# michiyasunaga/qagnn

Hardware: AMD Instinct MI355X
Metric: QA-subgraphs/sec (batch x num_choice) fwd+bwd (higher is better)
Workload: dtype f32; 1 GPU; configs[1]: CSQA-shaped batch 64 questions x 5 choices = 320 subgraphs per GPU, n=200 node slots, 400..2000 edges/subgraph, 38 relations (run_qagnn__csqa.sh), 5-layer GAT d=200 H=4, QAGNN decoder fwd+bwd (LM encoder excluded: random sent_vecs), dropout 0.2, train-mode BN; subgraphs_per_gpu=320, nodes=64000, edges=396800, edges_with_self_loops=460800, graph_input=load-time int32 blobs (qagnn_graph_from_blobs), 13.3 B/edge on the wire, parallelism=single

## Files before the change

__graft_entry__.py:

```python
import os
import sys

ROOT = os.path.dirname(os.path.abspath(__file__))
if ROOT not in sys.path:
    sys.path.insert(0, ROOT)


def build():
    from qagnn_amd.build import build as build_lib
    path = build_lib(force=False)
    from qagnn_amd import _lib
    lib = _lib.load_library(path)
    assert lib.qagnn_abi_version() == _lib.ABI_VERSION
    for name in _lib.EXPORTS + _lib.EXPORTS_TN + _lib.EXPORTS_INFER + _lib.EXPORTS_LOSS + _lib.EXPORTS_EXPLAIN:
        assert hasattr(lib, name), name
    import qagnn_amd.modeling_qagnn
    import oracle.qagnn_oracle
    print(f'[build] {path} ok ({os.path.getsize(path)} bytes), {len(_lib.EXPORTS)} C-ABI symbols')


def smoke():
    import torch
    sys.path.insert(0, os.path.join(ROOT, 'tests'))
    import helpers
    from qagnn_amd import modeling_qagnn as MQ
    from qagnn_amd import ops
    assert torch.cuda.is_available(), 'smoke() needs an MI355X'
    torch.set_num_threads(min(os.cpu_count() or 1, 32))
    case = dict(shape='config1', nq=1, nc=5, n=100, n_rel=17, std=0.6, train=True, seed=3,
                cfg=helpers.model_cfg(d=200, k=5, sent_dim=64, n_concept=1000, concept_in_dim=32))
    cfg = case['cfg']
    inp = helpers.make_case_inputs(case)
    B, n = 5, 100
    args = [inp['sent_vecs'], inp['concept_ids'].view(B, n), inp['node_type_ids'].view(B, n), inp['node_scores'].view(B, n, 1),
            inp['adj_lengths'].view(B), inp['edge_index'], inp['edge_type']]
    torch.manual_seed(0)
    model = MQ.QAGNN(None, cfg['k'], 4, 38, cfg['sent_dim'], cfg['n_concept'], 200, cfg['concept_in_dim'], 2, 200, 0, 0.0, 0.0, 0.0)
    helpers.det_fill_(model, 3, 0.6)
    model.pooler.dropout.p = model.pooler.attention.dropout.p = 0.0
    model = model.train().to('cuda:0')
    dargs = [a.to('cuda:0') for a in args]
    with helpers.recorded_forward(cfg['concept_dim']) as relu_in:
        logits, attn = model(*dargs[:5], (dargs[5], dargs[6]))
    (logits * torch.linspace(0.5, 1.5, B, device='cuda:0').view(B, 1)).sum().backward()
    assert ops.kernels().name == 'hip'
    ref = helpers.F64Ref(case, 'grad', inputs=tuple(args))
    ref.compute_yard()
    dl = helpers._close(logits.detach().cpu(), ref.forward32['::logits'], rtol=1e-4, atol=1e-5, what='logits')
    da = helpers._close(attn.detach().cpu(), ref.forward32['::pool_attn'], rtol=1e-4, atol=1e-5, what='pool_attn')
    report = ref.check_all({k: p.grad for k, p in model.named_parameters() if p.grad is not None}, what='smoke grad::', min_checked=60,
                           **helpers.kink_args(relu_in, cfg, args[5], args[6], args[2]))
    worst = max(report, key=report.get)
    print(f'[smoke] logits max|d| = {dl:.3e}, pool_attn max|d| = {da:.3e}; {len(report)} gradient tensors on the float64 yardstick, '
          f'worst {report[worst]:.2e} of scale ({worst})')


if __name__ == '__main__':
    build()
    if len(sys.argv) > 1 and sys.argv[1] == 'smoke':
        smoke()
```

qagnn_amd/_lib.py:

```python
import ctypes as C
import functools
import os

import torch

_HERE = os.path.dirname(os.path.abspath(__file__))
LIB_PATH = os.environ.get('QAGNN_LIB') or os.path.join(_HERE, 'libqagnn_hip.so')

EXPORTS = ['qagnn_last_error', 'qagnn_abi_version', 'qagnn_graph_storage_elems', 'qagnn_graph_prep', 'qagnn_graph_prep_blocked',
           'qagnn_graph_from_blobs', 'qagnn_radam_step_f32', 'qagnn_node_prep_f32', 'qagnn_seed_epoch_advance', 'qagnn_seed_epoch_set',
           'qagnn_gemm_nn_f32', 'qagnn_gemm_nn_split_f32', 'qagnn_gemm_nn_pack_bytes', 'qagnn_gemm_nn_ws_bytes', 'qagnn_gemm_nn_split_ws_f32', 'qagnn_gemm_nn_prepack_bytes', 'qagnn_gemm_nn_prepack_f32',
           'qagnn_gemm_nn_prepack_clear', 'qagnn_gemm_tn_workspace_elems', 'qagnn_gemm_tn_f32', 'qagnn_gemm_tn2_f32', 'qagnn_gemm_tn_colsum_f32',
           'qagnn_colreduce_workspace_elems', 'qagnn_colreduce_f32', 'qagnn_bn_finalize_f32', 'qagnn_bn_stats_finalize_f32', 'qagnn_bn_relu_bwd_f32',
           'qagnn_gelu_dropout_fwd_f32', 'qagnn_gelu_dropout_bwd_f32', 'qagnn_sin_basis_f32',
           'qagnn_bn_relu_bwd_colsum_f32',
           'qagnn_pool_attn_fwd_f32', 'qagnn_pool_attn_bwd_f32', 'qagnn_head_post_fwd_f32', 'qagnn_head_post_bwd_f32', 'qagnn_add_row0_f32', 'qagnn_gather_multi_f32', 'qagnn_gather_multi_sum_f32',
           'qagnn_edge_attn_fwd_f32', 'qagnn_edge_attn_bwd_f32',
           'qagnn_hop_fwd_workspace_elems', 'qagnn_hop_bwd_workspace_elems', 'qagnn_hop_fwd_f32', 'qagnn_hop_bwd_f32',
           'qagnn_stack_fwd_f32', 'qagnn_stack_bwd_f32', 'qagnn_absmax_f32', 'qagnn_zero_words', 'qagnn_gemm_tn_h2_f32', 'qagnn_gelu_dropout_fwd_amax_f32', 'qagnn_gelu_dropout_amax_scratch_elems',
           'qagnn_timing_enable', 'qagnn_timing_read', 'qagnn_gemm_tn_h1_f32', 'qagnn_gelu_dropout_bwd_amax_f32', 'qagnn_packed_min_rows',
           'qagnn_radam_step_scaled_f32', 'qagnn_grad_norm_workspace_elems', 'qagnn_grad_norm_f32', 'qagnn_scale_multi_f32', 'qagnn_graph_prep_cap',
           'qagnn_store_gather', 'qagnn_graph_from_store']
EXPORTS_TN = ['qagnn_gemm_tn_graph_f32', 'qagnn_gemm_tn_route_query', 'qagnn_tn_work_table', 'qagnn_tn_live_tiles']
EXPORTS_INFER = ['qagnn_infer_version', 'qagnn_bn_relu_absmax_scratch_elems', 'qagnn_bn_relu_absmax_f32', 'qagnn_stack_infer_f32',
                 'qagnn_choice_eval_f32']
EXPORTS_LOSS = ['qagnn_loss_version', 'qagnn_choice_loss_f32', 'qagnn_choice_loss_bwd_f32']
EXPORTS_EXPLAIN = ['qagnn_explain_version', 'qagnn_attn_export_f32', 'qagnn_attn_trace_f32']
TRACE_MAX_N = 1024
LOSS_KINDS = {'cross_entropy': 0, 'margin_rank': 1}
LOSS_THREADS = 256

CLS_SLICES = 4
ABI_VERSION = 25

_i32, _i64, _f32, _u64, _vp = C.c_int32, C.c_int64, C.c_float, C.c_uint64, C.c_void_p


class qagnn_graph(C.Structure):
    _fields_ = ([(n, _i32) for n in ('N', 'E', 'Ep', 'R', 'T', 'C')] +
                [(n, _vp) for n in ('rowptr_s', 'tgt_s', 'src_s', 'cls_s', 'eid_s', 'rowptr_t', 'src_t', 'tgt_t', 'cls_t', 'pos_t',
                                    'cls_count', 'src_c', 'tgt_c', 'pos_c', 'chunk_cls', 'chunk_beg',
                                    'chunk_len', 'n_chunks', 'chunkptr')] +
                [('max_chunks', _i32), ('err', _vp), ('block_n', _i32), ('n_groups', _i32)])


class qagnn_store(C.Structure):
    _fields_ = ([(n, _vp) for n in ('blobs', 'blob_off', 'concept_ids', 'node_type', 'node_scores', 'adj_len')] +
                [('S', _i32), ('n', _i32), ('W', _i64)])


GATHER_MAX = 160


class qagnn_gather_tabs(C.Structure):
    _fields_ = [('p', _vp * GATHER_MAX), ('n', _i32)]


class qagnn_pack_desc(C.Structure):
    _fields_ = [('B1n', _vp), ('ldn1', _i32), ('K1', _i32), ('B2n', _vp), ('ldn2', _i32), ('K2', _i32), ('No', _i32), ('pieces', _i32)]


class qagnn_gemm_nn_args(C.Structure):
    _fields_ = [('A1', _vp), ('lda1', _i32), ('K1', _i32), ('B1', _vp), ('ldb1', _i32),
                ('A2', _vp), ('lda2', _i32), ('K2', _i32), ('B2', _vp), ('ldb2', _i32),
                ('C', _vp), ('ldc', _i32), ('M', _i32), ('No', _i32),
                ('bias', _vp), ('rowtab', _vp), ('ldt', _i32), ('rowidx', _vp),
                ('a_scale', _vp), ('a_shift', _vp), ('accumulate', _i32), ('a_rowidx', _vp), ('xcd_remap', _i32), ('colstat_part', _vp),
                ('a_amax1', _vp), ('a_amax2', _vp), ('a_rows', _i64), ('pieces', _i32)]


class qagnn_hop_args(C.Structure):
    _fields_ = ([('g', C.POINTER(qagnn_graph))] + [(n, _i32) for n in ('N', 'DP', 'SP', 'HP', 'T')] + [('qscale', _f32)] +
                [(n, _vp) for n in ('X', 'S', 'ntype', 'Wx_t', 'Wx', 'Ws_t', 'Ws', 'TT', 'EkEm', 'W1t', 'W1', 'b1', 'gamma', 'beta',
                                    'W2t', 'W2', 'b2')] +
                [('batch_stats', _i32), ('eps', _f32), ('run_mean_p', _vp), ('run_var_p', _vp), ('run_mean', _vp), ('run_var', _vp),
                 ('num_batches_tracked', _vp), ('dense_pos', _vp), ('d', _i32), ('momentum', _f32),
                 ('apply_act', _i32), ('p_drop', _f32), ('seed', _u64)] +
                [(n, _vp) for n in ('KMQ', 'a', 'alpha', 'aggr', 'h1', 'out', 'y', 'stats', 'dy', 'dX', 'dS')] +
                [('accumulate_dS', _i32), ('accumulate_dX', _i32)] +
                [(n, _vp) for n in ('dWx_t', 'dWs_t', 'dTT', 'dEkEm', 'dW1t', 'db1', 'dbn', 'dW2t', 'db2', 'ws')] +
                [('ws_elems', _i64), ('gemm_split', _i32), ('ones_col', _i32), ('tab_col', _i32), ('side_stream', _vp), ('amax', _vp), ('x_amax', _vp), ('s_amax', _vp)])


HOP_AMAX_WORDS = 16
HOP_AM_X, HOP_AM_S, HOP_AM_AGGR, HOP_AM_H1, HOP_AM_Y, HOP_AM_DOUT, HOP_AM_DH1, HOP_AM_DKMQ = range(8)


def load_library(path=LIB_PATH):
    if not os.path.exists(path):
        raise OSError(f'{path} not found: build it with `python -m qagnn_amd.build` (hipcc, gfx950)')
    lib = C.CDLL(path)
    lib.qagnn_last_error.restype = C.c_char_p
    lib.qagnn_abi_version.restype = _i32
    lib.qagnn_graph_storage_elems.restype = _i64
    lib.qagnn_graph_storage_elems.argtypes = [_i32, _i32, _i32, _i32]
    lib.qagnn_graph_prep.argtypes = [C.POINTER(qagnn_graph), _vp, _vp, _vp, _vp, _i32, _i32, _i32, _i32, _vp]
    lib.qagnn_graph_prep_blocked.argtypes = [C.POINTER(qagnn_graph), _vp, _vp, _vp, _vp, _i32, _i32, _i32, _i32, _i32, _vp]
    lib.qagnn_graph_prep_cap.argtypes = [C.POINTER(qagnn_graph), _vp, _vp, _i64, _vp, _vp, _i32, _i32, _vp, _i32, _i32, _i32, _vp]
    lib.qagnn_graph_from_blobs.argtypes = [C.POINTER(qagnn_graph), _vp, _vp, _vp, _vp, _vp, _i32, _i32, _i32, _i32, _i32, _vp]
    lib.qagnn_store_gather.argtypes = [C.POINTER(qagnn_store), _vp, _i32, _vp, _vp, _vp, _vp, _vp, _vp, _vp]
    lib.qagnn_graph_from_store.argtypes = [C.POINTER(qagnn_graph), _vp, C.POINTER(qagnn_store), _vp, _vp, _vp, _i32, _i32, _i32, _i32, _vp]
    lib.qagnn_node_prep_f32.argtypes = [_vp, _vp, _vp, _vp, _i32, _i32, _vp, _vp, _vp, _i64, _vp, _vp]
    lib.qagnn_seed_epoch_advance.argtypes = [_u64, _vp]
    lib.qagnn_seed_epoch_set.argtypes = [_u64, _vp]
    lib.qagnn_radam_step_f32.argtypes = [_i32, _vp, _vp, _vp, _vp, _vp] + [C.c_double] * 6 + [_i32, _vp]
    lib.qagnn_radam_step_scaled_f32.argtypes = [_i32, _vp, _vp, _vp, _vp, _vp] + [C.c_double] * 6 + [_i32, _vp, _vp]
    lib.qagnn_grad_norm_workspace_elems.restype = _i64
    lib.qagnn_grad_norm_workspace_elems.argtypes = [_i32, _vp]
    lib.qagnn_grad_norm_f32.argtypes = [_i32, _vp, _vp, C.c_double, _vp, _vp, _vp]
    lib.qagnn_scale_multi_f32.argtypes = [_i32, _vp, _vp, _vp, _vp]
    lib.qagnn_gemm_nn_f32.argtypes = [C.POINTER(qagnn_gemm_nn_args), _vp]
    lib.qagnn_gemm_nn_split_f32.argtypes = [C.POINTER(qagnn_gemm_nn_args), _vp, _i32, _vp, _i32, _vp]
    lib.qagnn_gemm_nn_pack_bytes.restype = _i64
    lib.qagnn_gemm_nn_pack_bytes.argtypes = [_i32, _i32, _i32]
    lib.qagnn_gemm_nn_split_ws_f32.argtypes = [C.POINTER(qagnn_gemm_nn_args), _vp, _i32, _vp, _i32, _vp, _i64, _vp]
    lib.qagnn_gemm_nn_ws_bytes.restype = _i64
    lib.qagnn_gemm_nn_ws_bytes.argtypes = [C.POINTER(qagnn_gemm_nn_args), _vp, _i32, _vp, _i32]
    lib.qagnn_gemm_nn_prepack_bytes.restype = _i64
    lib.qagnn_gemm_nn_prepack_bytes.argtypes = [C.POINTER(qagnn_pack_desc), _i32]
    lib.qagnn_gemm_nn_prepack_f32.argtypes = [C.POINTER(qagnn_pack_desc), _i32, _vp, _i64, _i64, _vp]
    lib.qagnn_gemm_nn_prepack_clear.argtypes = [_i64]
    lib.qagnn_gemm_tn_workspace_elems.restype = _i64
    lib.qagnn_gemm_tn_workspace_elems.argtypes = [_i32, _i32, _i32]
    lib.qagnn_gemm_tn_f32.argtypes = [_vp, _i32, _vp, _i32, _vp, _i32, _i32, _i32, _i32, _vp, _vp, _vp, _i32, _vp, _vp]
    lib.qagnn_gemm_tn2_f32.argtypes = [_vp, _i32, _i32, _vp, _i32, _i32, _vp, _i32, _vp, _i32, _i32, _i32, _vp, _vp]
    lib.qagnn_gemm_tn_h2_f32.argtypes = [_vp, _i32, _i32, _vp, _i32, _i32, _vp, _i32, _vp, _i32, _i32, _i32, _vp, _vp, _vp, _vp, _vp, _vp, _vp]
    lib.qagnn_gemm_tn_h1_f32.argtypes = lib.qagnn_gemm_tn_h2_f32.argtypes
    lib.qagnn_gemm_tn_graph_f32.argtypes = [_vp, _i32, _i32, _vp, _i32, _i32, _vp, _i32, _vp, _i32, _i32, _i32, _vp, _vp, _vp, _i32,
                                            C.POINTER(qagnn_graph), _vp, _vp]
    lib.qagnn_gemm_tn_route_query.argtypes = [_i32, _i32, _i32, _i32, _vp]
    lib.qagnn_tn_work_table.argtypes = [C.POINTER(qagnn_graph), _i32, _i32, _vp, _vp]
    lib.qagnn_tn_live_tiles.argtypes = [_i32]
    lib.qagnn_absmax_f32.argtypes = [_vp, _i64, _vp, _vp]
    lib.qagnn_zero_words.argtypes = [_vp, _i64, _vp]
    lib.qagnn_timing_enable.argtypes = [_i32]
    lib.qagnn_timing_read.argtypes = [_vp, _vp]
    lib.qagnn_packed_min_rows.restype = _i64
    lib.qagnn_packed_min_rows.argtypes = [_i64]
    lib.qagnn_gemm_tn_colsum_f32.argtypes = [_vp, _i32, _vp, _i32, _vp, _i32, _i32, _i32, _i32, _vp, _vp, _vp, _i32, _vp, _vp, _i32,
                                             _vp, _vp]
    lib.qagnn_colreduce_workspace_elems.restype = _i64
    lib.qagnn_colreduce_workspace_elems.argtypes = [_i32, _i32, _i32]
    lib.qagnn_colreduce_f32.argtypes = [_i32, _vp, _i32, _vp, _i32, _i32, _i32, _vp, _i32, _vp, _vp, _vp, _vp, _vp, _f32, _vp, _vp, _vp]
    lib.qagnn_bn_finalize_f32.argtypes = [_vp, _vp, _vp, _vp, _f32, _vp, _vp, _vp, _i32, _vp, _vp, _vp, _vp, _i32, _f32, _f32, _i32, _vp]
    lib.qagnn_bn_stats_finalize_f32.argtypes = [_vp, _i32, _i32, _i32, _vp, _vp, _f32, _vp, _vp, _vp, _vp, _vp, _i32, _f32, _f32, _i32, _vp]
    lib.qagnn_bn_relu_bwd_f32.argtypes = [_vp, _vp, _vp, _i32, _i32, _i32, _vp, _vp, _vp, _vp, _vp, _vp, _vp, _f32, _vp, _vp]
    lib.qagnn_gelu_dropout_fwd_f32.argtypes = [_vp, _vp, _i64, _f32, _u64, _vp]
    lib.qagnn_gelu_dropout_bwd_f32.argtypes = [_vp, _vp, _vp, _i64, _f32, _u64, _vp]
    lib.qagnn_gelu_dropout_fwd_amax_f32.argtypes = [_vp, _vp, _i64, _f32, _u64, _vp, _vp, _vp]
    lib.qagnn_gelu_dropout_bwd_amax_f32.argtypes = [_vp, _vp, _vp, _i64, _f32, _u64, _vp, _vp, _vp]
    lib.qagnn_gelu_dropout_amax_scratch_elems.restype = _i64
    lib.qagnn_gelu_dropout_amax_scratch_elems.argtypes = [_i64]
    lib.qagnn_sin_basis_f32.argtypes = [_vp, _vp, _vp, _i32, _i32, _i32, _vp]
    lib.qagnn_bn_relu_bwd_colsum_f32.argtypes = [_vp, _vp, _vp, _i32, _i32, _i32, _vp, _vp, _vp, _vp, _vp, _vp, _vp, _f32, _vp, _vp, _vp, _vp]
    lib.qagnn_pool_attn_fwd_f32.argtypes = [_vp, _vp, _vp, _i32, _vp, _i32, _i32, _i32, _i32, _f32, _f32, _u64, _vp, _vp, _vp, _vp]
    lib.qagnn_pool_attn_bwd_f32.argtypes = [_vp, _vp, _i32, _i32, _i32, _i32, _i32, _f32, _f32, _u64, _vp, _vp, _vp, _vp, _vp, _i32, _vp, _vp, _vp]
    lib.qagnn_head_post_fwd_f32.argtypes = [_vp, _vp, _vp, _vp, _vp, _vp, _i64, _vp, _vp, _i32, _i32, _i32, _i32, _i32, _i32, _i32, _f32, _f32, _u64, _u64,
                                            _vp, _vp, _vp, _vp]
    lib.qagnn_head_post_bwd_f32.argtypes = [_vp, _vp, _vp, _vp, _vp, _vp, _vp, _i64, _vp, _i32, _i32, _i32, _i32, _i32, _i32, _i32, _f32, _f32, _u64, _u64,
                                            _vp, _vp, _vp, _vp, _vp, _vp, _i32, _vp]
    lib.qagnn_add_row0_f32.argtypes = [_vp, _i64, _vp, _i32, _i32, _vp]
    lib.qagnn_gather_multi_f32.argtypes = [C.POINTER(qagnn_gather_tabs), _vp, _vp, _vp, _i32, _vp]
    lib.qagnn_gather_multi_sum_f32.argtypes = [C.POINTER(qagnn_gather_tabs), _vp, _vp, _i32, _i32, _vp, _vp]
    lib.qagnn_edge_attn_fwd_f32.argtypes = [C.POINTER(qagnn_graph), _vp, _i32, _vp, _i32, _i32, _f32, _vp, _vp, _vp, _vp, _i32, _vp]
    lib.qagnn_edge_attn_bwd_f32.argtypes = [C.POINTER(qagnn_graph), _vp, _i32, _vp, _i32, _i32, _f32, _vp, _vp, _vp, _i32,
                                            _vp, _vp, _vp, _vp, _vp, _vp]
    lib.qagnn_hop_fwd_workspace_elems.restype = _i64
    lib.qagnn_hop_fwd_workspace_elems.argtypes = [_i32, _i32, _i32]
    lib.qagnn_hop_bwd_workspace_elems.restype = _i64
    lib.qagnn_hop_bwd_workspace_elems.argtypes = [_i32, _i32, _i32, _i32, _i32]
    lib.qagnn_hop_fwd_f32.argtypes = [C.POINTER(qagnn_hop_args), _vp]
    lib.qagnn_hop_bwd_f32.argtypes = [C.POINTER(qagnn_hop_args), _vp]
    lib.qagnn_stack_fwd_f32.argtypes = [C.POINTER(qagnn_hop_args), _i32, _vp]
    lib.qagnn_stack_bwd_f32.argtypes = [C.POINTER(qagnn_hop_args), _i32, _vp]
    lib.qagnn_infer_version.argtypes = []
    lib.qagnn_bn_relu_absmax_scratch_elems.restype = _i64
    lib.qagnn_bn_relu_absmax_scratch_elems.argtypes = [_i32, _i32]
    lib.qagnn_bn_relu_absmax_f32.argtypes = [_vp, _i32, _i32, _i32, _vp, _vp, _vp, _vp, _vp]
    lib.qagnn_stack_infer_f32.argtypes = [C.POINTER(qagnn_hop_args), _i32, _vp]
    lib.qagnn_choice_eval_f32.argtypes = [_vp, _i64, _vp, _i32, _i32, _vp, _vp, _vp]
    lib.qagnn_loss_version.argtypes = []
    lib.qagnn_choice_loss_f32.argtypes = [_vp, _i64, _vp, _i32, _i32, _i32, _f32, _vp, _vp, _vp, _i64, _vp, _vp, _vp]
    lib.qagnn_choice_loss_bwd_f32.argtypes = [_vp, _i64, _vp, _vp, _i64, _i32, _i32, _vp]
    lib.qagnn_explain_version.argtypes = []
    lib.qagnn_attn_export_f32.argtypes = [C.POINTER(qagnn_graph), _vp, _i64, _i32, _vp, _i64, _vp]
    lib.qagnn_attn_trace_f32.argtypes = [C.POINTER(qagnn_graph), _vp, _i64, _i32, _i32, _i32, _i32, _i32, _vp, _vp, _vp, _vp]
    for name in EXPORTS + EXPORTS_TN + EXPORTS_INFER + EXPORTS_LOSS + EXPORTS_EXPLAIN:
        fn = getattr(lib, name)
        if fn.restype is C.c_int and name not in ('qagnn_abi_version',):
            fn.restype = _i32
    return lib


def _ptr(t):
    return None if t is None else t.data_ptr()


def choice_loss_bound(kind, nc, Q, max_abs=1.0, margin=0.0, weight=1.0, threads=LOSS_THREADS):
    import math
    u, v = 2.0 ** -24, 2.0 ** -53
    M, L, w = max(1.0, float(max_abs)), math.log(nc), abs(float(weight))
    S = -(-Q // threads) + math.log2(threads) + nc
    if LOSS_KINDS[kind] == 0:
        return w * M * (u * (nc + 8 + 5 * L) + v * S * (2 + L)), w / Q * u * (nc + 8 + L)
    return w * M * (3 * u + v * S) * (2 + abs(float(margin)) / M), w / Q * 2 * u


def _running_fields(running):
    if running is None:
        return None, None, None, None, 0, 0.0, 1.0
    rm, rv, nbt, pos, mom, unb = running
    assert rm.is_contiguous() and rv.is_contiguous() and pos.dtype == torch.long and (nbt is None or nbt.dtype == torch.long)
    return rm.data_ptr(), rv.data_ptr(), _ptr(nbt), pos.data_ptr(), rm.numel(), float(mom), float(unb)


def _chk2d(t, name, dtype=torch.float32):
    assert t.is_cuda and t.dtype == dtype and t.dim() == 2 and t.is_contiguous(), \
        f'{name}: need a contiguous 2-D {dtype} device tensor, got {tuple(t.shape)} {t.dtype} {t.device}'
    return t


def _chkp(t, name):
    assert t.is_cuda and t.dtype == torch.float32 and t.dim() == 2, f'{name}: need a 2-D float32 device tensor, got {tuple(t.shape)} {t.dtype} {t.device}'
    assert t.is_contiguous() or (t.stride(1) == 1 and (t.size(0) == 1 or (t.stride(0) >= t.size(1) and t.stride(0) % 4 == 0)) and t.data_ptr() % 16 == 0), \
        f'{name}: rows must be contiguous, a multiple of 4 floats (and at least their width) apart and 16-byte aligned; got strides {t.stride()} for {tuple(t.shape)}'
    return t


def _ld(t):
    return t.size(1) if t.size(0) == 1 else t.stride(0)


def _chkp3(t, name):
    assert t.is_cuda and t.dtype == torch.float32 and t.dim() == 3, f'{name}: need a 3-D float32 device tensor'
    B, n, Cc = t.shape
    ld = _ld3(t)
    assert t.is_contiguous() or (t.stride(2) == 1 and ld >= Cc and ld % 4 == 0 and (B == 1 or t.stride(0) == n * ld) and t.data_ptr() % 16 == 0), \
        f'{name}: need [B, n, Cc] rows with one pitch (a multiple of 4 floats, >= Cc), 16-byte aligned; got strides {t.stride()} for {tuple(t.shape)}'
    return t


def _ld3(t):
    B, n, Cc = t.shape
    return t.stride(1) if n > 1 else (t.stride(0) if B > 1 else Cc)


VALIDATE = os.environ.get('QAGNN_VALIDATE', '0') == '1'


class _ErrWatch:

    def __init__(self):
        self.pending = []
        self.sink = None

    def watch(self, flags, what, reset=None):
        if torch.cuda.is_current_stream_capturing():
            if self.sink is not None:
                self.sink.append((flags, what, reset))
            return
        self.after_replay([(flags, what, reset)])

    def after_replay(self, watched):
        for flags, what, reset in watched:
            host = torch.empty(4, dtype=torch.int32, pin_memory=True)
            host.copy_(flags, non_blocking=True)
            ev = torch.cuda.Event()
            ev.record()
            self.pending.append((ev, host, what, reset))
        if VALIDATE:
            self.poll(block=True)

    def poll(self, block=False):
        if torch.cuda.is_available() and torch.cuda.is_current_stream_capturing():
            return
        keep, bad = [], None
        for ev, host, what, reset in self.pending:
            if block:
                ev.synchronize()
            if not ev.query():
                keep.append((ev, host, what, reset))
            elif int(host[0]) != 0:
                if reset is not None:
                    reset.zero_()
                if bad is None:
                    bad = what
        self.pending = keep
        if bad is not None:
            raise RuntimeError(f'out-of-range input in {bad}: the device replaced it by a safe value; the results of that batch '
                               'are not the reference\'s (which raises in its one-hot / index ops)')


ERR_WATCH = _ErrWatch()


class HipGraph:

    def __init__(self, storage, cstruct, N, E, R, T, block_n=0):
        self.storage, self.c = storage, cstruct
        self.N, self.E, self.Ep, self.R, self.T = N, E, E + N, R, T
        self.block_n = block_n
        self.dynamic = False
        self.C = R * T * T + T
        self.max_chunks = cstruct.max_chunks

    def array(self, name, length):
        off = (getattr(self.c, name) - self.storage.data_ptr()) // 4
        return self.storage[off:off + length]

    def live_tiles(self):
        T = (self.N + 31) // 32
        T4 = (T + 3) // 4 * 4
        w = self.array('err', 16 + 4 + 2 * T4)[16:]
        return w[4:4 + T], w[4 + T4:4 + T4 + T], w[:1]

    @property
    def cls_part_rows(self):
        return self.max_chunks + CLS_SLICES * self.C

    @property
    def cls_count(self):
        return self.array('cls_count', self.C)

    @property
    def eid_s(self):
        return self.array('eid_s', self.Ep)


def _device_of(args, kwargs):
    for a in list(args) + list(kwargs.values()):
        if isinstance(a, torch.Tensor):
            if a.is_cuda:
                return a.device
        elif isinstance(a, HipGraph):
            return a.storage.device
        elif isinstance(a, (tuple, list)):
            for t in a:
                if isinstance(t, torch.Tensor) and t.is_cuda:
                    return t.device
    return None


def _on_operand_device(fn):
    @functools.wraps(fn)
    def wrapped(self, *args, **kwargs):
        dev = _device_of(args, kwargs)
        if dev is None or dev.index == torch.cuda.current_device():
            return fn(self, *args, **kwargs)
        with torch.cuda.device(dev):
            return fn(self, *args, **kwargs)
    return wrapped


class _GuardedMeta(type):
    def __new__(mcls, name, bases, ns):
        for k, v in list(ns.items()):
            if callable(v) and not k.startswith('_'):
                ns[k] = _on_operand_device(v)
        return super().__new__(mcls, name, bases, ns)


class HipKernels(metaclass=_GuardedMeta):
    name = 'hip'
    infer_attn = True
    tn_live = True

    def __init__(self):
        if not torch.cuda.is_available():
            raise RuntimeError('qagnn_amd needs an MI355X: torch.cuda.is_available() is False and there is no CPU fallback')
        self.lib = load_library()
        if self.lib.qagnn_abi_version() != ABI_VERSION:
            raise RuntimeError('libqagnn_hip.so ABI version mismatch')
        self.gemm_split = {'0': 0, '1': 1, '3': 3}.get(os.environ.get('QAGNN_GEMM_SPLIT', '2'), 2)
        self.PACK_MIN_M = int(self.lib.qagnn_packed_min_rows(-1))
        self._side_streams = {}
        self._loss_flags = {}

    def _stream(self):
        return torch._C._cuda_getCurrentRawStream(torch.cuda.current_device())

    def _side_stream(self):
        dev = torch.cuda.current_device()
        st = self._side_streams.get(dev)
        if st is None:
            st = self._side_streams[dev] = torch.cuda.Stream(device=dev)
        return st.cuda_stream

    def _check(self, rc, what):
        if rc != 0:
            raise RuntimeError(f'{what} failed (code {rc}): {self.lib.qagnn_last_error().decode()}')

    def _graph_alloc(self, N, E, R, T, device, storage=None):
        elems = self.lib.qagnn_graph_storage_elems(N, E, R, T)
        if storage is None:
            storage = torch.empty(elems, dtype=torch.int32, device=device)
        assert storage.is_cuda and storage.dtype == torch.int32 and storage.is_contiguous() and storage.numel() >= elems
        return storage, qagnn_graph()
# ... 804 lines not shown
        self._check_scale_word(grad_out, g.device)
        Q, nc = g.shape
        if out is None:
            out = torch.empty((Q, nc), dtype=torch.float32, device=g.device)
        assert out.dtype == torch.float32 and out.shape == (Q, nc) and out.device == g.device and (out.stride(1) == 1 or nc == 1)
        self._check(self.lib.qagnn_choice_loss_bwd_f32(g.data_ptr(), _ld(g), grad_out.data_ptr(), out.data_ptr(), _ld(out), Q, nc, self._stream()),
                    'qagnn_choice_loss_bwd_f32')
        return out

    def stack_infer(self, graph, HP, qscale, X, S, ntype, prms, eps, cols=-1, x_amax=None, s_amax=None, keep=False, attn=False):
        assert not (keep and attn)
        k = len(prms)
        N, DP, Ep, dev = graph.N, 4 * HP, graph.Ep, X.device
        kk = k if keep else 1
        KMQ = torch.empty((kk, N, 3 * DP), dtype=torch.float32, device=dev)
        aa = torch.empty((kk, 2, Ep, 4), dtype=torch.float32, device=dev)
        rows = torch.empty((kk, 4, N, DP), dtype=torch.float32, device=dev) if keep else torch.empty((5, N, DP), dtype=torch.float32, device=dev)
        stats = torch.empty((kk, 5, DP), dtype=torch.float32, device=dev)
        amax = torch.empty((k, HOP_AMAX_WORDS), dtype=torch.int32, device=dev)
        ws = self._fwd_ws(graph, DP, dev)
        ys = [rows[l, 3] if keep else rows[3 + (l & 1)] for l in range(k)]
        hops = self._hop_chain(graph, HP, qscale, X, S, ntype, prms, ys, (KMQ, aa, rows, stats), amax.data_ptr(), x_amax, s_amax, ws, False, eps, 0.0,
                               None, cols, shared=not keep)
        if attn:
            a_all = torch.empty((k, Ep, 4), dtype=torch.float32, device=dev)
            for l in range(k):
                hops[l].a = a_all.data_ptr() + l * Ep * 16
        self._check(self.lib.qagnn_stack_infer_f32(hops, k, self._stream()), 'qagnn_stack_infer_f32')
        if attn:
            return ys[-1], amax, a_all
        return (ys[-1], amax, (KMQ, aa, rows, stats)) if keep else (ys[-1], amax)

    @staticmethod
    def _chk_attn(graph, a):
        assert a.is_cuda and a.dtype == torch.float32 and a.dim() == 3 and a.shape[1:] == (graph.Ep, 4), \
            f'a: need a [k, Ep = {graph.Ep}, 4] float32 device tensor, got {tuple(a.shape)} {a.dtype} {a.device}'
        k = a.size(0)
        ls = a.stride(0) if k > 1 else 4 * graph.Ep
        assert k == 0 or ((graph.Ep == 1 or a.stride(1) == 4) and a.stride(2) == 1 and ls >= 4 * graph.Ep and ls % 4 == 0 and a.data_ptr() % 16 == 0), \
            f'a: rows of 4 contiguous floats, layers a multiple of 4 floats apart, 16-byte aligned; got strides {a.stride()}'
        return k, ls

    def attn_export(self, graph, a, out=None):
        k, ls = self._chk_attn(graph, a)
        if out is None:
            out = torch.empty((k, graph.Ep, 4), dtype=torch.float32, device=a.device)
        ko, ols = self._chk_attn(graph, out)
        assert ko == k and out.device == a.device
        self._check(self.lib.qagnn_attn_export_f32(C.byref(graph.c), a.data_ptr() if k else None, ls, k, out.data_ptr() if k else None, ols,
                                                   self._stream()), 'qagnn_attn_export_f32')
        return out

    def attn_trace(self, graph, a, B, n, root=0, head=-1, out=None):
        k, ls = self._chk_attn(graph, a)
        N, dev = graph.N, a.device
        if out is None:
            out = (torch.empty((k + 1, N), dtype=torch.float32, device=dev), torch.empty((k + 1, N), dtype=torch.float32, device=dev),
                   torch.empty((k, N), dtype=torch.int32, device=dev))
        flow, best, pred = out
        for t, rows, dt in ((flow, k + 1, torch.float32), (best, k + 1, torch.float32), (pred, k, torch.int32)):
            assert t.is_cuda and t.dtype == dt and t.shape == (rows, N) and t.is_contiguous() and t.device == dev
        self._check(self.lib.qagnn_attn_trace_f32(C.byref(graph.c), a.data_ptr() if k else None, ls, k, int(B), int(n), int(root), int(head),
                                                  flow.data_ptr(), best.data_ptr(), pred.data_ptr() if k else None, self._stream()),
                    'qagnn_attn_trace_f32')
        return flow, best, pred

    def stack_fwd(self, graph, HP, qscale, X, S, ntype, prms, batch_stats, eps, p, seeds, runnings, cols=-1, x_amax=None, s_amax=None):
        k = len(prms)
        N, DP, Ep, dev = graph.N, 4 * HP, graph.Ep, X.device
        KMQ = torch.empty((k, N, 3 * DP), dtype=torch.float32, device=dev)
        aa = torch.empty((k, 2, Ep, 4), dtype=torch.float32, device=dev)
        rows = torch.empty((k, 4, N, DP), dtype=torch.float32, device=dev)
        stats = torch.empty((k, 5, DP), dtype=torch.float32, device=dev)
        amax = torch.empty((k, HOP_AMAX_WORDS), dtype=torch.int32, device=dev)
        ws = self._fwd_ws(graph, DP, dev)
        ys = rows[:, 3].unbind(0)
        hops = self._hop_chain(graph, HP, qscale, X, S, ntype, prms, ys, (KMQ, aa, rows, stats), amax.data_ptr(), x_amax, s_amax, ws, batch_stats, eps, p,
                               seeds, cols, runnings=runnings)
        self._check(self.lib.qagnn_stack_fwd_f32(hops, k, self._stream()), 'qagnn_stack_fwd_f32')
        ext = torch.empty(0, dtype=torch.int32, device=dev)
        return ys[k - 1], (KMQ, aa, rows, stats, amax, x_amax if x_amax is not None else ext, s_amax if s_amax is not None else ext)

    def stack_bwd(self, graph, HP, qscale, X, S, ntype, prms, batch_stats, eps, p, seeds, saved, dy, need_dX, need_dS, dX_acc=None, tab_col=-1,
                  overlap=True):
        k = len(prms)
        KMQ, aa, rows, stats = saved[:4]
        p_amax = saved[4].data_ptr() if len(saved) > 4 else None
        x_amax, s_amax = (saved[5], saved[6]) if len(saved) > 6 else (None, None)
        N, DP, Ep, dev = graph.N, 4 * HP, graph.Ep, X.device
        SP = S.size(1) if S is not None else 0
        _chk2d(dy, 'dy')
        sizes, offs = self._grad_sizes(DP, SP, prms[0][4].size(0), graph.C)
        per = offs[-1]
        flat = torch.empty(k * per, dtype=torch.float32, device=dev)
        dxs = torch.empty((max(k - 1, 1), N, DP), dtype=torch.float32, device=dev)
        dS = torch.empty((N, SP), dtype=torch.float32, device=dev) if (SP and need_dS) else None
        dX = None
        if need_dX:
            dX = dX_acc if dX_acc is not None else torch.empty((N, DP), dtype=torch.float32, device=dev)
            assert dX.shape == (N, DP) and dX.is_contiguous()
        ws = self._bwd_ws(graph, DP, SP, dev)
        hops = self._hop_chain(graph, HP, qscale, X, S, ntype, prms, rows[:, 3].unbind(0), (KMQ, aa, rows, stats), p_amax, x_amax, s_amax, ws,
                               batch_stats, eps, p, seeds, tab_col, side=overlap)
        grads, p_dxs, row_b = [], dxs.data_ptr(), N * DP * 4
        for l, h in enumerate(hops):
            h.dy = dy.data_ptr() if l == k - 1 else p_dxs + l * row_b
            grads.append(self._carve_grads(h, flat[l * per:(l + 1) * per], sizes, offs, graph.C))
            if l > 0:
                h.dX, h.accumulate_dX = p_dxs + (l - 1) * row_b, 0
            elif dX is not None:
                h.dX, h.accumulate_dX = dX.data_ptr(), (1 if dX_acc is not None else 0)
            if dS is not None:
                h.dS, h.accumulate_dS = dS.data_ptr(), (0 if l == k - 1 else 1)
        self._check(self.lib.qagnn_stack_bwd_f32(hops, k, self._stream()), 'qagnn_stack_bwd_f32')
        return dX, dS, grads
```

qagnn_amd/build.py:

```python
import hashlib
import os
import subprocess
import sys

HERE = os.path.dirname(os.path.abspath(__file__))
CSRC = os.path.join(HERE, 'csrc')
LIB = os.path.join(HERE, 'libqagnn_hip.so')
STAMP = LIB + '.srchash'
SOURCES = ['graph_prep.hip', 'gemm.hip', 'elementwise.hip', 'edge_attn.hip', 'pool.hip', 'hop.hip', 'optim.hip', 'gemm_split.hip', 'gemm_nn2.hip', 'gemm_dispatch.hip', 'timing.hip', 'infer.hip', 'loss.hip', 'explain.hip']
FLAGS = ['--offload-arch=gfx950', '-O3', '-std=c++17', '-fPIC', '-shared']


def hashed_files():
    headers = sorted(f for f in os.listdir(CSRC) if f.endswith('.h'))
    return [os.path.join(CSRC, s) for s in SOURCES + headers] + [os.path.join(HERE, '..', 'include', 'qagnn_hip.h'),
                                                                 os.path.join(HERE, '..', 'include', 'qagnn_hip_tn.h'),
                                                                 os.path.join(HERE, '..', 'include', 'qagnn_hip_infer.h'),
                                                                 os.path.join(HERE, '..', 'include', 'qagnn_hip_loss.h'),
                                                                 os.path.join(HERE, '..', 'include', 'qagnn_hip_explain.h')]


def source_hash():
    h = hashlib.sha256(' '.join(FLAGS).encode())
    for p in hashed_files():
        with open(p, 'rb') as f:
            h.update(os.path.basename(p).encode() + b'\0' + f.read() + b'\0')
    return h.hexdigest()


def up_to_date():
    if not (os.path.exists(LIB) and os.path.exists(STAMP)):
        return False
    with open(STAMP) as f:
        return f.read().strip() == source_hash()


def build(force=False, verbose=True):
    if not force and up_to_date():
        return LIB
    hipcc = os.environ.get('HIPCC', '/opt/rocm/bin/hipcc')
    cmd = [hipcc] + FLAGS + ['-o', LIB] + [os.path.join(CSRC, s) for s in SOURCES]
    if verbose:
        print(' '.join(cmd), flush=True)
    if os.path.exists(STAMP):
        os.remove(STAMP)
    subprocess.check_call(cmd)
    with open(STAMP, 'w') as f:
        f.write(source_hash() + '\n')
    return LIB


if __name__ == '__main__':
    print(build(force='--force' in sys.argv))
```

qagnn_amd/csrc/common.h:

```cpp
#pragma once
#include <hip/hip_runtime.h>
#include <stdint.h>
#include <stdio.h>

#include <type_traits>

#include "../../include/qagnn_hip.h"
#include "../../include/qagnn_hip_tn.h"
#include "../../include/qagnn_hip_infer.h"

namespace qagnn {

void set_error(const char* fmt, ...);

struct NnProduct {
  const qagnn_gemm_nn_args* a;
  bool split;
  const float* B1n; int ldn1; const float* B2n; int ldn2;
  void* ws; int64_t ws_bytes;
};
enum class NnFamily { FP32, SPLIT, NN2 };
enum class NnB { IN_KERNEL, PACK, IMAGE };
struct NnRoute {
  NnFamily family;
// ... 36 lines not shown
  const float* a_scale; const float* a_shift; const int64_t* a_rowidx; int accumulate;
  float* bsum; const int64_t* b_rowidx; int groups;
  const uint32_t* amax[3]; int np;
  float* ws;
  const qagnn_graph* g;
};
inline TnProduct tn_product(const float* A1, int lda1, int Ka1, const float* A2, int lda2, int Ka2, const float* B, int ldb, float* C, int ldc, int R,
                            int No, const float* a_scale, const float* a_shift, float* ws, const uint32_t* amax_a1 = nullptr,
                            const uint32_t* amax_a2 = nullptr, const uint32_t* amax_b = nullptr, int np = 3) {
  TnProduct p = {};
  p.A1 = A1; p.lda1 = lda1; p.Ka1 = Ka1;
  if (A2 && Ka2 > 0) { p.A2 = A2; p.lda2 = lda2; p.Ka2 = Ka2; p.two = true; }
  p.B = B; p.ldb = ldb; p.C = C; p.ldc = ldc; p.R = R; p.No = No; p.a_scale = a_scale; p.a_shift = a_shift; p.ws = ws;
  p.amax[0] = amax_a1; p.amax[1] = amax_a2; p.amax[2] = amax_b; p.np = np;
  return p;
}
enum class TnFamily { RUNTIME, STRIP, SPLIT, WS, PAIR };
struct TnRoute {
  TnFamily family;
  int kt, nt, waves, np;
  bool affine, gather, colsum;
  int chunk_rows, nchunks;
  bool sum_by4;
  bool live;
  dim3 grid;
  int64_t ws_elems;
};
TnRoute tn_route(const TnProduct& p);
int gemm_tn(const TnProduct& p, hipStream_t stream);
int launch_tn(const TnRoute& r, const TnProduct& p, float* Pcs, hipStream_t stream);
int launch_tn_strip(const TnRoute& r, const TnProduct& p, float* Pcs, hipStream_t stream);
int launch_tn_split(const TnRoute& r, const TnProduct& p, hipStream_t stream);
int launch_tn_ws(const TnRoute& r, const TnProduct& p, hipStream_t stream);
int launch_sum_chunks(const float* P, float* C, int ldc, int rows, int No, int nchunks, int accumulate, bool by4, hipStream_t stream);

constexpr int TN_LIST_CAP = 1024;
constexpr int TN_LIVE_BC = 208;
struct TnLive { const int* list; const int* n_live; int T, S, chunk_tiles; };
struct TnWork { int cK, cM, lenM, qK, rK; };
struct TnSlot { int cb, list, beg, cnt, pslot; };
__host__ __device__ inline TnWork tn_work(int S, int T, int L, int chunk_tiles) {
  TnWork w;
  L = L < 0 ? 0 : (L > T ? T : L);
  if (L >= T) {
    w.cK = S / 3; w.cM = S - 2 * w.cK; w.lenM = chunk_tiles; w.qK = -1; w.rK = 0;
    return w;
  }
  const long long den = (long long)T + 2ll * L;
  int c = (int)((2ll * S * L + den) / (2 * den));
  const int hi = (S - 1) / 2;
  c = c < 1 ? 1 : (c > hi ? hi : c);
  w.cK = c; w.cM = S - 2 * c; w.lenM = (T + w.cM - 1) / w.cM; w.qK = L / c; w.rK = L % c;
  return w;
}
__host__ __device__ inline TnSlot tn_slot(const TnWork& w, int S, int T, int u) {
  auto start = [&](int j) { return 2 * j + (int)((long long)j * w.cM / w.cK); };
  int j = (int)((long long)u * w.cK / S);
  while (j > 0 && start(j) > u) --j;
  while (j + 1 < w.cK && start(j + 1) <= u) ++j;
  const int off = u - start(j);
  TnSlot s;
  auto range = [&](int i) { s.list = 0; s.beg = i * w.lenM < T ? i * w.lenM : T; s.cnt = T - s.beg < w.lenM ? T - s.beg : w.lenM; };
  if (off < 2) {
    s.cb = off == 0 ? 0 : 2;
    s.pslot = off == 0 ? j : w.cK + j;
    if (w.qK < 0) range(j);
    else { s.list = 1; s.beg = j * w.qK + (j < w.rK ? j : w.rK); s.cnt = w.qK + (j < w.rK ? 1 : 0); }
  } else {
    const int m = (int)((long long)j * w.cM / w.cK) + off - 2;
    s.cb = 1;
    s.pslot = 2 * w.cK + m;
    range(m);
  }
  return s;
}
int launch_sum_chunks_live(const float* P, float* C, int ldc, int rows, const TnLive& lv, int accumulate, hipStream_t stream);
bool tn_live_enabled();
struct LiveTiles { int n_tiles; int32_t *n_live, *live, *list; };
inline LiveTiles live_tiles_of(const qagnn_graph* g) {
  const int T = (int)(((int64_t)g->N + 31) / 32), T4 = (T + 3) & ~3;
  int32_t* const p = g->err + 16;
  return LiveTiles{T, p, p + 4, p + 4 + T4};
}

int launch_gelu_dropout(const float* X, const float* dY, float* out, int64_t n, float p, uint64_t seed, uint32_t* amax, float* amax_part,
                        hipStream_t stream);
int64_t gelu_amax_scratch_elems(int64_t n);
int launch_bn_relu_bwd_colsum(const float* dR, const float* Hh, float* dH, int ld, int R, int Cc, const float* mean, const float* invstd,
                              const float* scale, const float* shift, const float* gamma, const float* sum_dy, const float* sum_dy_hhat,
                              float inv_rows, const float* roww, float* colsum, float* workspace, uint32_t* amax, hipStream_t stream);
int launch_bn_stats_finalize(const float* part, int n_tiles, int R, int Cc, const float* gamma, const float* beta, float eps, float* stats,
                             float* run_mean, float* run_var, int64_t* nbt, int d, float momentum, float unbias, int ones_col, uint32_t* amax_bound,
                             hipStream_t stream);

int launch_edge_attn_fwd(const qagnn_graph* g, const float* KMQ, int32_t ldk, const float* EkEm, int32_t lde, int32_t HP, float qscale,
                         float* score, float* a, float* alpha, float* aggr, int32_t lda, float* amax_part , hipStream_t stream);
int launch_edge_attn_bwd(const qagnn_graph* g, const float* KMQ, int32_t ldk, const float* EkEm, int32_t lde, int32_t HP, float qscale,
                         const float* a, const float* alpha, const float* G, int32_t ldg, float* dKMQ, float* dEkEm, float* ga, float* rs,
                         float* cls_part, float* amax_part , uint32_t* amax_slot, hipStream_t stream);
int launch_amax_reduce(const float* part, int64_t n, uint32_t* slot, hipStream_t stream);
int launch_bn_relu_absmax(const float* H, int ldh, int R, int Cc, const float* scale, const float* shift, uint32_t* slot, float* part, hipStream_t stream);

struct TimedScope {
  int kind;
  hipStream_t s;
  hipEvent_t e0, e1;
  bool counted;
  TimedScope(int kind, hipStream_t s);
  ~TimedScope();
  TimedScope(const TimedScope&) = delete;
  TimedScope& operator=(const TimedScope&) = delete;
};

#define QAGNN_REQUIRE(cond, code, ...) \
  do {                                 \
    if (!(cond)) {                     \
      qagnn::set_error(__VA_ARGS__);   \
      return (code);                   \
    }                                  \
  } while (0)

#define QAGNN_LAUNCH_CHECK(name)                                               \
  do {                                                                         \
    hipError_t e__ = hipGetLastError();                                        \
    if (e__ != hipSuccess) {                                                   \
      qagnn::set_error("%s launch failed: %s", name, hipGetErrorString(e__));  \
      return QAGNN_EHIP;                                                       \
    }                                                                          \
  } while (0)

#ifndef QAGNN_NN_OCC
#define QAGNN_NN_OCC 2
#endif

template <int V0, int... Vs, class F>
inline int dispatch_int(int v, F&& f) {
  if constexpr (sizeof...(Vs) == 0) return f(std::integral_constant<int, V0>{});
  else return v == V0 ? f(std::integral_constant<int, V0>{}) : dispatch_int<Vs...>(v, f);
}
template <class F>
inline int dispatch_bool(bool v, F&& f) { return v ? f(std::true_type{}) : f(std::false_type{}); }

template <auto KERNEL>
inline int raise_lds_limit(int bytes, const char* name) {
  static bool raised[64] = {};
  int dev = 0;
  if (hipGetDevice(&dev) != hipSuccess) dev = 0;
  if (bytes <= 64 * 1024 || raised[dev & 63]) return QAGNN_OK;
  hipError_t e = hipFuncSetAttribute((const void*)KERNEL, hipFuncAttributeMaxDynamicSharedMemorySize, bytes);
  if (e != hipSuccess) { set_error("%s: cannot raise the dynamic LDS limit: %s", name, hipGetErrorString(e)); return QAGNN_EHIP; }
  raised[dev & 63] = true;
  return QAGNN_OK;
}

static inline bool aligned16(const void* p) { return (reinterpret_cast<uintptr_t>(p) & 15u) == 0; }

__device__ __forceinline__ int xcd_remap(int b, int nblocks) {
  const int q = nblocks >> 3, r = nblocks & 7;
  const int xcd = b & 7, slot = b >> 3;
  const int base = xcd < r ? xcd * (q + 1) : r * (q + 1) + (xcd - r) * q;
  return base + slot;
}

__host__ __device__ __forceinline__ int edge_xcd_cap(int N) {
  const int per = (((N + 3) >> 2) + 7) >> 3;
  return (per * 5 + 3) >> 2;
}
__device__ __forceinline__ int xcd_remap_balanced(int b, const int* __restrict__ base) {
  const int xcd = b & 7, lb = base[xcd] + (b >> 3);
  return lb < base[xcd + 1] ? lb : -1;
}

const unsigned long long* seed_epoch_ptr();
__device__ __forceinline__ uint64_t epoch_seed(uint64_t seed, const unsigned long long* __restrict__ epoch) {
  return epoch ? seed + (uint64_t)epoch[0] * 0xD1B54A32D192ED03ull : seed;
}

__device__ __forceinline__ float uniform01(uint64_t seed, uint64_t idx) {
  uint64_t z = seed + (idx + 1) * 0x9E3779B97F4A7C15ull;
  z = (z ^ (z >> 30)) * 0xBF58476D1CE4E5B9ull;
  z = (z ^ (z >> 27)) * 0x94D049BB133111EBull;
  z = z ^ (z >> 31);
// ... 121 lines not shown
```

qagnn_amd/csrc/edge_attn.hip:

```cpp
#include "common.h"

namespace qagnn {

#ifndef EDGE_UNROLL
#define EDGE_UNROLL 4
#endif
#define TGT_UNROLL 4

typedef __amdgpu_buffer_rsrc_t rsrc_t;
constexpr uint32_t OOB_OFF = 0x7FFFFFF0u;
__device__ __forceinline__ rsrc_t make_rsrc(const void* base, uint32_t bytes) {
  return __builtin_amdgcn_make_buffer_rsrc(const_cast<void*>(base), 0, (int)bytes, 0x00020000);
}
__device__ __forceinline__ float4 buf_ld4(rsrc_t r, uint32_t voff, uint32_t soff) {
  return __builtin_bit_cast(float4, __builtin_amdgcn_raw_buffer_load_b128(r, (int)voff, (int)soff, 0));
}

constexpr int SLAB_ROWS = 72;

struct Lane {
  int lane, w, g, j;
  bool act;
  uint32_t voff;
  int off;
// ... 270 lines not shown
  const int s = wave_node(xcd_base);
  if (s >= N) return;
  const Lane L = lane_info(HP);
  const int DP = 4 * HP;
  const uint32_t pk = (uint32_t)ldk * 4u, pe = (uint32_t)lde * 4u;
  const rsrc_t rK = make_rsrc(KMQ, (uint32_t)N * pk), rE = make_rsrc(EkEm, (uint32_t)C * pe);
  const int beg = __builtin_amdgcn_readfirstlane(rowptr_s[s]), end = __builtin_amdgcn_readfirstlane(rowptr_s[s + 1]);
  if (end - beg == 1) {
    if (L.act) st4(dKMQ + (int64_t)s * ldk + 2 * DP + L.off, zero4());
    if (amax_part && L.lane == 63) amax_part[s] = 0.f;
    return;
  }
  const float4 r4 = ld4(rs + (int64_t)s * 4);
  slab_init(slab[L.w], L.lane);
  const float* const sl = reinterpret_cast<const float*>(slab[L.w]) + L.g;
  float4 dQ = zero4();
  for (int e0 = beg; e0 < end; e0 += 64) {
    const int cnt = min(64, end - e0), lc = e0 + min(L.lane, cnt - 1);
    const uint32_t tv = (uint32_t)tgt_s[lc] * pk, cv = (uint32_t)cls_s[lc] * pe;
    float4 gs4 = zero4();
    if (L.lane < cnt) {
      const float4 a4 = ld4(a + (int64_t)lc * 4), g4 = ld4(ga + (int64_t)lc * 4);
      gs4 = make_float4(qscale * a4.x * (g4.x - r4.x), qscale * a4.y * (g4.y - r4.y), qscale * a4.z * (g4.z - r4.z),
                        qscale * a4.w * (g4.w - r4.w));
      st4(ga + (int64_t)lc * 4, gs4);
    }
    slab[L.w][L.lane] = gs4;
    for (int i = 0; i < cnt; i += EDGE_UNROLL) {
      float4 k[EDGE_UNROLL], ek[EDGE_UNROLL];
#pragma unroll
      for (int u = 0; u < EDGE_UNROLL; ++u) {
        const int idx = min(i + u, cnt - 1);
        k[u] = buf_ld4(rK, L.voff, rl(tv, idx));
        ek[u] = buf_ld4(rE, L.voff, rl(cv, idx));
      }
#pragma unroll
      for (int u = 0; u < EDGE_UNROLL; ++u) dQ = fma4(sl[(i + u) * 4], add4(k[u], ek[u]), dQ);
    }
  }
  if (L.act) st4(dKMQ + (int64_t)s * ldk + 2 * DP + L.off, dQ);
  if (amax_part) node_amax(L.act ? absmax4(dQ) : 0.f, amax_part, s);
}

__global__ __launch_bounds__(256) void k_edge_bwd_tgt(const int* __restrict__ rowptr_t, const int* __restrict__ src_t,
                                                      const int* __restrict__ pos_t, const float* __restrict__ KMQ, int ldk,
                                                      int HP, const float* __restrict__ gsb, float* __restrict__ dKMQ, int N,
                                                      const int* __restrict__ xcd_base, float* __restrict__ amax_part) {
  __shared__ float4 slab[4][SLAB_ROWS];
  const int t = wave_node(xcd_base);
  if (t >= N) return;
  const Lane L = lane_info(HP);
  const int DP = 4 * HP;
  const uint32_t pk = (uint32_t)ldk * 4u, vq = L.voff + 2u * DP * 4u;
  const rsrc_t rK = make_rsrc(KMQ, (uint32_t)N * pk);
  const int beg = __builtin_amdgcn_readfirstlane(rowptr_t[t]), end = __builtin_amdgcn_readfirstlane(rowptr_t[t + 1]);
  if (end - beg == 1) {
    const int sv = __builtin_amdgcn_readfirstlane(src_t[beg]), pv = __builtin_amdgcn_readfirstlane(pos_t[beg]);
    const float4 q1 = buf_ld4(rK, vq, (uint32_t)sv * pk);
    const float gs1 = gsb[(int64_t)pv * 4 + L.g];
    const float4 k1 = fma4(gs1, q1, zero4());
    if (L.act) st4(dKMQ + (int64_t)t * ldk + L.off, k1);
    if (amax_part) node_amax(L.act ? absmax4(k1) : 0.f, amax_part, t);
    return;
  }
  slab_init(slab[L.w], L.lane);
  const float* const sl = reinterpret_cast<const float*>(slab[L.w]) + L.g;
  float4 dK = zero4();
  for (int e0 = beg; e0 < end; e0 += 64) {
    const int cnt = min(64, end - e0), lc = e0 + min(L.lane, cnt - 1);
    const uint32_t sv = (uint32_t)src_t[lc] * pk;
    slab[L.w][L.lane] = L.lane < cnt ? ld4(gsb + (int64_t)pos_t[lc] * 4) : zero4();
    for (int i = 0; i < cnt; i += TGT_UNROLL) {
      float4 qv[TGT_UNROLL];
#pragma unroll
      for (int u = 0; u < TGT_UNROLL; ++u) qv[u] = buf_ld4(rK, vq, rl(sv, min(i + u, cnt - 1)));
#pragma unroll
      for (int u = 0; u < TGT_UNROLL; ++u) dK = fma4(sl[(i + u) * 4], qv[u], dK);
    }
  }
  if (L.act) st4(dKMQ + (int64_t)t * ldk + L.off, dK);
  if (amax_part) node_amax(L.act ? absmax4(dK) : 0.f, amax_part, t);
}

__global__ __launch_bounds__(256) void k_edge_bwd_cls(const int* __restrict__ n_chunks, const int* __restrict__ chunk_beg,
                                                      const int* __restrict__ chunk_len, const int* __restrict__ src_c,
                                                      const int* __restrict__ tgt_c, const int* __restrict__ pos_c,
                                                      const float* __restrict__ KMQ, int ldk, int HP,
                                                      const float* __restrict__ alpha, const float* __restrict__ gsb,
                                                      const float* __restrict__ G, int ldg, float* __restrict__ cls_part, int N) {
  __shared__ float4 slab[2][4][SLAB_ROWS];
  const int nch = *n_chunks, nb_real = (nch + 3) >> 2;
  if ((int)blockIdx.x >= nb_real) return;
  const int k = __builtin_amdgcn_readfirstlane(xcd_remap(blockIdx.x, nb_real) * 4 + (threadIdx.x >> 6));
  if (k >= nch) return;
  const Lane L = lane_info(HP);
  const int DP = 4 * HP;
  const uint32_t pk = (uint32_t)ldk * 4u, pg = (uint32_t)ldg * 4u, vq = L.voff + 2u * DP * 4u;
  const rsrc_t rK = make_rsrc(KMQ, (uint32_t)N * pk), rG = make_rsrc(G, (uint32_t)N * pg);
  const int beg = __builtin_amdgcn_readfirstlane(chunk_beg[k]), len = __builtin_amdgcn_readfirstlane(chunk_len[k]);
  slab_init(slab[0][L.w], L.lane);
  slab_init(slab[1][L.w], L.lane);
  const float* const sl_gs = reinterpret_cast<const float*>(slab[0][L.w]) + L.g;
  const float* const sl_al = reinterpret_cast<const float*>(slab[1][L.w]) + L.g;
  float4 dEk = zero4(), dEm = zero4();
  for (int b0 = 0; b0 < len; b0 += 64) {
    const int cnt = min(64, len - b0), lc = beg + b0 + min(L.lane, cnt - 1);
    const uint32_t sv = (uint32_t)src_c[lc] * pk, tv = (uint32_t)tgt_c[lc] * pg;
    const int pv = pos_c[lc];
    slab[0][L.w][L.lane] = L.lane < cnt ? ld4(gsb + (int64_t)pv * 4) : zero4();
    slab[1][L.w][L.lane] = L.lane < cnt ? ld4(alpha + (int64_t)pv * 4) : zero4();
    for (int i = 0; i < cnt; i += EDGE_UNROLL) {
      float4 qv[EDGE_UNROLL], g4[EDGE_UNROLL];
#pragma unroll
      for (int u = 0; u < EDGE_UNROLL; ++u) {
        const int idx = min(i + u, cnt - 1);
        qv[u] = buf_ld4(rK, vq, rl(sv, idx));
        g4[u] = buf_ld4(rG, L.voff, rl(tv, idx));
      }
#pragma unroll
      for (int u = 0; u < EDGE_UNROLL; ++u) {
        dEk = fma4(sl_gs[(i + u) * 4], qv[u], dEk);
        dEm = fma4(sl_al[(i + u) * 4], g4[u], dEm);
      }
    }
  }
  if (L.act) {
    st4(cls_part + (int64_t)k * 2 * DP + L.off, dEk);
    st4(cls_part + (int64_t)k * 2 * DP + DP + L.off, dEm);
  }
}

__global__ __launch_bounds__(1024) void k_cls_reduce(const int* __restrict__ chunkptr, const float* __restrict__ cls_part,
                                                     float* __restrict__ slices, int DP2, int C, int NG) {
  extern __shared__ float4 sm4[];
  __shared__ int cp_lo[QAGNN_CLS_GROUPS], cp_hi[QAGNN_CLS_GROUPS];
  const int c = blockIdx.x, sl = blockIdx.y;
  if (threadIdx.x < NG) {
    cp_lo[threadIdx.x] = chunkptr[threadIdx.x * C + c];
    cp_hi[threadIdx.x] = chunkptr[threadIdx.x * C + c + 1];
  }
  __syncthreads();
  const int ncol4 = DP2 >> 2;
  const int P = (int)blockDim.x / ncol4;
  const int col4 = threadIdx.x % ncol4, part = threadIdx.x / ncol4;
  float4 acc = zero4();
  if (part < P) {
    int seen = 0;
    for (int g = sl; g < NG; g += QAGNN_CLS_SLICES) {
      const int kb = cp_lo[g], ke = cp_hi[g];
      const int first = (part - seen % P + P) % P;
      for (int k = kb + first; k < ke; k += P) acc = add4(acc, ld4(cls_part + (int64_t)k * DP2 + col4 * 4));
      seen += ke - kb;
    }
    sm4[part * ncol4 + col4] = acc;
  }
  __syncthreads();
  if (threadIdx.x < ncol4) {
    float4 s = sm4[threadIdx.x];
    for (int q = 1; q < P; ++q) s = add4(s, sm4[q * ncol4 + threadIdx.x]);
    st4(slices + ((int64_t)c * QAGNN_CLS_SLICES + sl) * DP2 + threadIdx.x * 4, s);
  }
}
__global__ __launch_bounds__(256) void k_cls_reduce2(const float* __restrict__ slices, float* __restrict__ dEkEm, int lde, int DP2, int C,
                                                     const float* __restrict__ amax_part, int npart, uint32_t* __restrict__ amax_slot) {
  const int ncol4 = DP2 >> 2;
  const int i = blockIdx.x * blockDim.x + threadIdx.x;
  if (i < C * ncol4) {
    const int c = i / ncol4, col4 = i - c * ncol4;
    const float* p = slices + (int64_t)c * QAGNN_CLS_SLICES * DP2 + col4 * 4;
    float4 s = ld4(p);
#pragma unroll
    for (int q = 1; q < QAGNN_CLS_SLICES; ++q) s = add4(s, ld4(p + (int64_t)q * DP2));
    st4(dEkEm + (int64_t)c * lde + col4 * 4, s);
  }
  if (amax_part) {
    __shared__ float red[16];
    float m = 0.f;
    for (int k = i; k < npart; k += (int)(gridDim.x * blockDim.x)) m = fmaxf(m, amax_part[k]);
    block_amax_merge(m, amax_slot, red);
  }
}

static int check_common(const qagnn_graph* g, const float* KMQ, int ldk, const float* EkEm, int lde, int HP, const char* who) {
  QAGNN_REQUIRE(g && KMQ && EkEm, QAGNN_EINVAL, "%s: null pointer", who);
  QAGNN_REQUIRE(HP > 0 && HP % 4 == 0 && HP <= 64, QAGNN_EUNSUPPORTED, "%s: head pitch HP=%d must be a multiple of 4, <= 64", who, HP);
  QAGNN_REQUIRE(ldk >= 12 * HP && ldk % 4 == 0 && lde >= 8 * HP && lde % 4 == 0, QAGNN_EINVAL, "%s: ldk=%d lde=%d too small for HP=%d",
                who, ldk, lde, HP);
  QAGNN_REQUIRE(aligned16(KMQ) && aligned16(EkEm), QAGNN_EINVAL, "%s: operands must be 16-byte aligned", who);
  QAGNN_REQUIRE((int64_t)g->N * ldk * 4 < (int64_t)OOB_OFF && (int64_t)g->C * lde * 4 < (int64_t)OOB_OFF, QAGNN_EUNSUPPORTED,
                "%s: N=%d x ldk=%d floats exceed the 2 GiB a buffer descriptor of these kernels addresses", who, g->N, ldk);
  return QAGNN_OK;
}

}

using namespace qagnn;

namespace qagnn {
int launch_edge_attn_fwd(const qagnn_graph* g, const float* KMQ, int32_t ldk, const float* EkEm, int32_t lde, int32_t HP, float qscale,
                         float* score, float* a, float* alpha, float* aggr, int32_t lda, float* amax_part, hipStream_t stream) {
  TimedScope timed(2, stream);
  int rc = check_common(g, KMQ, ldk, EkEm, lde, HP, "edge_attn_fwd");
  if (rc != QAGNN_OK) return rc;
  QAGNN_REQUIRE(score && a && alpha && aggr && lda >= 4 * HP && lda % 4 == 0 && aligned16(aggr), QAGNN_EINVAL,
                "edge_attn_fwd: bad output arguments");
  const int nb = 8 * edge_xcd_cap(g->N);
  k_edge_scores<<<nb, 256, 0, stream>>>(g->rowptr_s, g->tgt_s, g->cls_s, KMQ, ldk, EkEm, lde, HP, qscale, score, a, alpha, g->N, g->C, g->err + 4);
  QAGNN_LAUNCH_CHECK("k_edge_scores");
  k_edge_aggregate<<<nb, 256, 0, stream>>>(g->rowptr_t, g->src_t, g->cls_t, g->pos_t, KMQ, ldk, EkEm, lde, HP, alpha, aggr, lda, g->N, g->C, g->err + 4, amax_part);
  QAGNN_LAUNCH_CHECK("k_edge_aggregate");
  return QAGNN_OK;
}
}

extern "C" int qagnn_edge_attn_fwd_f32(const qagnn_graph* g, const float* KMQ, int32_t ldk, const float* EkEm, int32_t lde,
                                       int32_t HP, float qscale, float* score, float* a, float* alpha, float* aggr, int32_t lda,
                                       qagnn_stream_t stream_) {
  return launch_edge_attn_fwd(g, KMQ, ldk, EkEm, lde, HP, qscale, score, a, alpha, aggr, lda, nullptr, (hipStream_t)stream_);
}

extern "C" int qagnn_edge_attn_bwd_f32(const qagnn_graph* g, const float* KMQ, int32_t ldk, const float* EkEm, int32_t lde,
                                       int32_t HP, float qscale, const float* a, const float* alpha, const float* G, int32_t ldg,
                                       float* dKMQ, float* dEkEm, float* ga, float* rs, float* cls_part, qagnn_stream_t stream_) {
  return launch_edge_attn_bwd(g, KMQ, ldk, EkEm, lde, HP, qscale, a, alpha, G, ldg, dKMQ, dEkEm, ga, rs, cls_part, nullptr, nullptr, (hipStream_t)stream_);
}

int qagnn::launch_edge_attn_bwd(const qagnn_graph* g, const float* KMQ, int32_t ldk, const float* EkEm, int32_t lde, int32_t HP, float qscale,
                                const float* a, const float* alpha, const float* G, int32_t ldg, float* dKMQ, float* dEkEm, float* ga, float* rs,
                                float* cls_part, float* amax_part, uint32_t* amax_slot, hipStream_t stream) {
  TimedScope timed(3, stream);
  int rc = check_common(g, KMQ, ldk, EkEm, lde, HP, "edge_attn_bwd");
  if (rc != QAGNN_OK) return rc;
  QAGNN_REQUIRE(a && alpha && G && dKMQ && dEkEm && ga && rs && cls_part, QAGNN_EINVAL, "edge_attn_bwd: null pointer");
  QAGNN_REQUIRE(ldg >= 4 * HP && ldg % 4 == 0 && aligned16(G) && aligned16(dKMQ) && aligned16(dEkEm) && aligned16(cls_part),
                QAGNN_EINVAL, "edge_attn_bwd: bad pitch / alignment");
  QAGNN_REQUIRE((int64_t)g->N * ldg * 4 < (int64_t)OOB_OFF, QAGNN_EUNSUPPORTED, "edge_attn_bwd: G exceeds 2 GiB");
  const int DP2 = 8 * HP;
  QAGNN_REQUIRE(DP2 / 4 <= 1024, QAGNN_EUNSUPPORTED, "edge_attn_bwd: HP too large");
  const int nb = 8 * edge_xcd_cap(g->N);
  k_edge_bwd_src1<<<nb, 256, 0, stream>>>(g->rowptr_s, g->tgt_s, g->cls_s, KMQ, ldk, EkEm, lde, HP, a, alpha, G, ldg, dKMQ, ga, rs, g->N, g->C, g->err + 4, amax_part);
  QAGNN_LAUNCH_CHECK("k_edge_bwd_src1");
  k_edge_bwd_src2<<<nb, 256, 0, stream>>>(g->rowptr_s, g->tgt_s, g->cls_s, KMQ, ldk, EkEm, lde, HP, qscale, a, dKMQ, ga, rs, g->N, g->C, g->err + 4, amax_part ? amax_part + g->N : nullptr);
  QAGNN_LAUNCH_CHECK("k_edge_bwd_src2");
  k_edge_bwd_tgt<<<nb, 256, 0, stream>>>(g->rowptr_t, g->src_t, g->pos_t, KMQ, ldk, HP, ga, dKMQ, g->N, g->err + 4, amax_part ? amax_part + 2 * (int64_t)g->N : nullptr);
  QAGNN_LAUNCH_CHECK("k_edge_bwd_tgt");
  k_edge_bwd_cls<<<cdiv(g->max_chunks, 4), 256, 0, stream>>>(g->n_chunks, g->chunk_beg, g->chunk_len, g->src_c, g->tgt_c, g->pos_c,
                                                             KMQ, ldk, HP, alpha, ga, G, ldg, cls_part, g->N);
  QAGNN_LAUNCH_CHECK("k_edge_bwd_cls");
  const int cr_threads = g->Ep < 65536 && DP2 / 4 <= 128 ? 256 : 1024;
  const int P = cr_threads / (DP2 / 4);
  float* slices = cls_part + (int64_t)g->max_chunks * DP2;
  k_cls_reduce<<<dim3(g->C, QAGNN_CLS_SLICES), cr_threads, (size_t)P * (DP2 / 4) * sizeof(float4), stream>>>(g->chunkptr, cls_part, slices, DP2,
                                                                                                          g->C, g->n_groups);
  QAGNN_LAUNCH_CHECK("k_cls_reduce");
  k_cls_reduce2<<<cdiv((int64_t)g->C * (DP2 / 4), 256), 256, 0, stream>>>(slices, dEkEm, lde, DP2, g->C, amax_slot ? amax_part : nullptr, 3 * g->N, amax_slot);
  QAGNN_LAUNCH_CHECK("k_cls_reduce2");
  return QAGNN_OK;
}
```

qagnn_amd/csrc/elementwise.hip:

```cpp
#include "common.h"

namespace qagnn {

constexpr int CR_WR_BIG = 32, CR_WR_SMALL = 8;
static inline int cr_wr(int R) { return R < 32768 ? CR_WR_SMALL : CR_WR_BIG; }

template <int MODE, int CR_WR>
__global__ __launch_bounds__(256) void k_colreduce(const float* __restrict__ X, int ldx, const float* __restrict__ X2, int ldx2,
                                                   int R, int Cc, const int64_t* __restrict__ rowidx, int groups,
                                                   const float* __restrict__ mean, const float* __restrict__ invstd,
                                                   const float* __restrict__ scale, const float* __restrict__ shift,
                                                   const float* __restrict__ roww, float* __restrict__ part) {
  constexpr int NOUT = MODE == 0 ? 4 : (MODE == 2 ? 2 : 1);
  __shared__ __attribute__((aligned(16))) float red[4][NOUT][256];
  const int lane = threadIdx.x & 63, w = threadIdx.x >> 6;
  const int col = blockIdx.x * 256 + lane * 4;
  const bool act = col < Cc;
  constexpr int CR_ROWS = 4 * CR_WR;
  const int r0 = blockIdx.y * CR_ROWS + w * CR_WR;
  float4 acc[NOUT];
#pragma unroll
  for (int o = 0; o < NOUT; ++o) acc[o] = make_float4(0.f, 0.f, 0.f, 0.f);
  float4 mu = make_float4(0.f, 0.f, 0.f, 0.f), is = mu, sc = mu, sh = mu;
  if (act && MODE >= 1) mu = ld4(mean + col);
  if (act && MODE == 2) { is = ld4(invstd + col); sc = ld4(scale + col); sh = ld4(shift + col); }
  if (act) {
    const int rend = min(R, r0 + CR_WR);
    for (int rb = r0; rb < rend; rb += 8) {
      float4 xs[8], hs[8];
#pragma unroll
      for (int u = 0; u < 8; ++u) {
        const int r = min(rb + u, rend - 1);
        xs[u] = ld4(X + (int64_t)r * ldx + col);
        if (MODE == 2) hs[u] = ld4(X2 + (int64_t)r * ldx2 + col);
      }
#pragma unroll
      for (int u = 0; u < 8; ++u) {
        const int r = rb + u;
        if (r >= rend) break;
        float4 x = xs[u];
        const float wr = (MODE != 2 && roww) ? roww[r] : 1.f;
        if (MODE == 0) {
          x = make_float4(x.x * wr, x.y * wr, x.z * wr, x.w * wr);
          const int g = rowidx ? (int)rowidx[r] : 0;
          if (g == 0) acc[0] = add4(acc[0], x);
          else if (g == 1) acc[1] = add4(acc[1], x);
          else if (g == 2) acc[2] = add4(acc[2], x);
          else acc[3] = add4(acc[3], x);
        } else if (MODE == 1) {
          const float4 d = make_float4(x.x - mu.x, x.y - mu.y, x.z - mu.z, x.w - mu.w);
          acc[0] = make_float4(fmaf(d.x * wr, d.x, acc[0].x), fmaf(d.y * wr, d.y, acc[0].y), fmaf(d.z * wr, d.z, acc[0].z),
                               fmaf(d.w * wr, d.w, acc[0].w));
        } else {
          const float4 h = hs[u];
          float4 dy;
          dy.x = fmaf(h.x, sc.x, sh.x) <= 0.f ? 0.f : x.x;
          dy.y = fmaf(h.y, sc.y, sh.y) <= 0.f ? 0.f : x.y;
          dy.z = fmaf(h.z, sc.z, sh.z) <= 0.f ? 0.f : x.z;
          dy.w = fmaf(h.w, sc.w, sh.w) <= 0.f ? 0.f : x.w;
          acc[0] = add4(acc[0], dy);
          acc[1].x = fmaf(dy.x, (h.x - mu.x) * is.x, acc[1].x);
          acc[1].y = fmaf(dy.y, (h.y - mu.y) * is.y, acc[1].y);
          acc[1].z = fmaf(dy.z, (h.z - mu.z) * is.z, acc[1].z);
          acc[1].w = fmaf(dy.w, (h.w - mu.w) * is.w, acc[1].w);
        }
      }
    }
  }
#pragma unroll
  for (int o = 0; o < NOUT; ++o) st4(&red[w][o][lane * 4], acc[o]);
  __syncthreads();
  const int nout = MODE == 0 ? groups : NOUT;
  for (int i = threadIdx.x; i < nout * 256; i += 256) {
    const int o = i >> 8, c = i & 255;
    if (blockIdx.x * 256 + c < Cc) {
      const float s = (red[0][o][c] + red[1][o][c]) + (red[2][o][c] + red[3][o][c]);
      part[((int64_t)blockIdx.y * nout + o) * Cc + blockIdx.x * 256 + c] = s;
    }
  }
}

constexpr int CF_Q = 16;
__global__ __launch_bounds__(64 * CF_Q) void k_colreduce_final(const float* __restrict__ part, float* __restrict__ out, int nchunks,
                                                               int tot, float out_scale) {
  __shared__ float red[CF_Q][64];
  const int lane = threadIdx.x & 63, q = threadIdx.x >> 6;
  const int o = blockIdx.x * 64 + lane;
  float s0 = 0.f, s1 = 0.f;
  if (o < tot) {
    int c = q;
#pragma unroll 4
    for (; c + CF_Q < nchunks; c += 2 * CF_Q) {
      s0 += part[(int64_t)c * tot + o];
      s1 += part[(int64_t)(c + CF_Q) * tot + o];
    }
    if (c < nchunks) s0 += part[(int64_t)c * tot + o];
  }
  red[q][lane] = s0 + s1;
  __syncthreads();
  if (q == 0 && o < tot) {
    float s = red[0][lane];
#pragma unroll
    for (int k = 1; k < CF_Q; ++k) s += red[k][lane];
    out[o] = s * out_scale;
  }
}


__global__ void k_bn_relu_bwd(const float* __restrict__ dR, const float* __restrict__ Hh, float* __restrict__ dH, int ld, int R,
                              int Cc, const float* __restrict__ mean, const float* __restrict__ invstd,
                              const float* __restrict__ scale, const float* __restrict__ shift, const float* __restrict__ gamma,
                              const float* __restrict__ sum_dy, const float* __restrict__ sum_dy_hhat, float inv_rows,
                              const float* __restrict__ roww) {
  const int c4n = Cc >> 2;
  const int64_t i = (int64_t)blockIdx.x * blockDim.x + threadIdx.x;
  if (i >= (int64_t)R * c4n) return;
  const int r = (int)(i / c4n), col = (int)(i % c4n) * 4;
  if (roww) inv_rows = roww[r];
  const int64_t off = (int64_t)r * ld + col;
  const float4 g = ld4(dR + off), h = ld4(Hh + off);
  const float4 mu = ld4(mean + col), is = ld4(invstd + col), sc = ld4(scale + col), sh = ld4(shift + col);
  const float4 ga = ld4(gamma + col), k1 = ld4(sum_dy + col), k2 = ld4(sum_dy_hhat + col);
  float4 o;
#define ONE(f)                                              \
  {                                                         \
    const float dy = fmaf(h.f, sc.f, sh.f) <= 0.f ? 0.f : g.f; \
    const float hh = (h.f - mu.f) * is.f;                   \
    o.f = ga.f * is.f * (dy - k1.f * inv_rows - hh * (k2.f * inv_rows)); \
  }
  ONE(x) ONE(y) ONE(z) ONE(w)
#undef ONE
  st4(dH + off, o);
}

__global__ void k_bn_finalize(const float* __restrict__ mean, const float* __restrict__ var, const float* __restrict__ gamma,
                              const float* __restrict__ beta, float eps, float* __restrict__ invstd, float* __restrict__ scale,
                              float* __restrict__ shift, int Cc, float* __restrict__ run_mean, float* __restrict__ run_var,
                              int64_t* __restrict__ nbt, const int64_t* __restrict__ dense_pos, int d, float momentum, float unbias,
                              int ones_col) {
  const int i = blockIdx.x * blockDim.x + threadIdx.x;
  if (i < Cc) {
    const float is = rsqrtf(var[i] + eps), sc = gamma[i] * is;
    invstd[i] = is;
    scale[i] = i == ones_col ? 0.f : sc;
    shift[i] = i == ones_col ? 1.f : beta[i] - mean[i] * sc;
  }
  if (run_mean && i < d) {
    const int64_t p = dense_pos[i];
    run_mean[i] += momentum * (mean[p] - run_mean[i]);
    run_var[i] += momentum * (var[p] * unbias - run_var[i]);
  }
  if (nbt && i == 0) *nbt += 1;
}

constexpr int ST_TILE = 128;
constexpr int BF_COLS = 16, BF_PARTS = 64;
struct Moments { float n, mean, m2; };
__device__ __forceinline__ void merge(Moments& a, float nb, float mb, float m2b) {
  if (nb <= 0.f) return;
  const float n = a.n + nb, d = mb - a.mean;
  a.mean += d * (nb / n);
  a.m2 += m2b + d * d * (a.n * nb / n);
  a.n = n;
}
__global__ __launch_bounds__(BF_COLS * BF_PARTS) void k_bn_stats_finalize(const float* __restrict__ part, int nt, int R, int Cc,
                                                                        const float* __restrict__ gamma, const float* __restrict__ beta,
                                                                        float eps, float* __restrict__ stats, float* __restrict__ run_mean,
                                                                        float* __restrict__ run_var, int64_t* __restrict__ nbt, int d,
                                                                        float momentum, float unbias, int ones_col,
                                                                        uint32_t* __restrict__ amax_bound) {
// ... 157 lines not shown
  }
        ONE(x) ONE(y) ONE(z) ONE(w)
#undef ONE
        asm volatile("" : "+v"(o.x), "+v"(o.y), "+v"(o.z), "+v"(o.w));
        st4(dH + (int64_t)r * ld + col, o);
        acc = add4(acc, o);
        am = fmaxf(am, absmax4(o));
      }
    }
  }
  st4(&red[w][lane * 4], acc);
  __syncthreads();
  const int c = threadIdx.x;
  if (blockIdx.x * 256 + c < Cc)
    part[(int64_t)blockIdx.y * Cc + blockIdx.x * 256 + c] = (red[0][c] + red[1][c]) + (red[2][c] + red[3][c]);
  if (amax) {
    __shared__ float ared[16];
    block_amax_merge(am, amax, ared);
  }
}

__device__ unsigned long long g_seed_epoch = 0;
__global__ void k_seed_epoch(unsigned long long* w, unsigned long long v, int add) { *w = add ? *w + v : v; }

const unsigned long long* seed_epoch_ptr() {
  static const unsigned long long* cache[64] = {};
  int dev = 0;
  if (hipGetDevice(&dev) != hipSuccess) dev = 0;
  const unsigned long long*& p = cache[dev & 63];
  if (!p) {
    void* a = nullptr;
    if (hipGetSymbolAddress(&a, HIP_SYMBOL(g_seed_epoch)) != hipSuccess) return nullptr;
    p = static_cast<const unsigned long long*>(a);
  }
  return p;
}

__global__ void k_sin_basis(const float* __restrict__ score, const float* __restrict__ js, float* __restrict__ out, int ldo, int R,
                            int J) {
  const int64_t i = (int64_t)blockIdx.x * blockDim.x + threadIdx.x;
  if (i >= (int64_t)R * ldo) return;
  const int r = (int)(i / ldo), j = (int)(i % ldo);
  out[i] = j < J ? sinf(js[j] * score[r]) : 0.f;
}

}

using namespace qagnn;

extern "C" int64_t qagnn_colreduce_workspace_elems(int32_t R, int32_t Cc, int32_t groups) {
  return (int64_t)cdiv(R, 4 * cr_wr(R)) * (groups < 2 ? 2 : groups) * Cc;
}

extern "C" int qagnn_colreduce_f32(int32_t mode, const float* X, int32_t ldx, const float* X2, int32_t ldx2, int32_t R, int32_t Cc,
                                   const int64_t* rowidx, int32_t groups, const float* mean, const float* invstd,
                                   const float* scale, const float* shift, const float* roww, float out_scale, float* out, float* workspace, qagnn_stream_t stream_) {
  hipStream_t stream = (hipStream_t)stream_;
  QAGNN_REQUIRE(X && out && workspace, QAGNN_EINVAL, "colreduce: null pointer");
  QAGNN_REQUIRE(R > 0 && Cc > 0 && Cc % 4 == 0 && ldx % 4 == 0 && aligned16(X), QAGNN_EINVAL, "colreduce: bad sizes/alignment");
  QAGNN_REQUIRE(mode >= 0 && mode <= 2, QAGNN_EINVAL, "colreduce: bad mode %d", mode);
  QAGNN_REQUIRE(ldx >= Cc && (mode != 2 || ldx2 >= Cc), QAGNN_EINVAL, "colreduce: ldx=%d / ldx2=%d below Cc=%d", ldx, ldx2, Cc);
  const bool small = cr_wr(R) == CR_WR_SMALL;
  dim3 grid(cdiv(Cc, 256), cdiv(R, 4 * cr_wr(R)));
  int nout;
  if (mode == 0) {
    QAGNN_REQUIRE(groups >= 1 && groups <= 4 && (groups == 1 || rowidx), QAGNN_EINVAL, "colreduce: groups=%d (1..4)", groups);
    nout = groups;
    if (small) k_colreduce<0, CR_WR_SMALL><<<grid, 256, 0, stream>>>(X, ldx, X2, ldx2, R, Cc, rowidx, groups, mean, invstd, scale, shift, roww, workspace);
    else k_colreduce<0, CR_WR_BIG><<<grid, 256, 0, stream>>>(X, ldx, X2, ldx2, R, Cc, rowidx, groups, mean, invstd, scale, shift, roww, workspace);
  } else if (mode == 1) {
    QAGNN_REQUIRE(mean && aligned16(mean), QAGNN_EINVAL, "colreduce: mode 1 needs mean");
    nout = 1;
    if (small) k_colreduce<1, CR_WR_SMALL><<<grid, 256, 0, stream>>>(X, ldx, X2, ldx2, R, Cc, rowidx, groups, mean, invstd, scale, shift, roww, workspace);
    else k_colreduce<1, CR_WR_BIG><<<grid, 256, 0, stream>>>(X, ldx, X2, ldx2, R, Cc, rowidx, groups, mean, invstd, scale, shift, roww, workspace);
  } else {
    QAGNN_REQUIRE(X2 && mean && invstd && scale && shift && ldx2 % 4 == 0 && aligned16(X2), QAGNN_EINVAL,
                  "colreduce: mode 2 needs X2, mean, invstd, scale, shift");
    nout = 2;
    if (small) k_colreduce<2, CR_WR_SMALL><<<grid, 256, 0, stream>>>(X, ldx, X2, ldx2, R, Cc, rowidx, groups, mean, invstd, scale, shift, roww, workspace);
    else k_colreduce<2, CR_WR_BIG><<<grid, 256, 0, stream>>>(X, ldx, X2, ldx2, R, Cc, rowidx, groups, mean, invstd, scale, shift, roww, workspace);
  }
  QAGNN_LAUNCH_CHECK("k_colreduce");
  const int tot = nout * Cc;
  k_colreduce_final<<<cdiv(tot, 64), 64 * CF_Q, 0, stream>>>(workspace, out, grid.y, tot, out_scale);
  QAGNN_LAUNCH_CHECK("k_colreduce_final");
  return QAGNN_OK;
}

extern "C" int qagnn_bn_relu_bwd_f32(const float* dR, const float* Hh, float* dH, int32_t ld, int32_t R, int32_t Cc,
                                     const float* mean, const float* invstd, const float* scale, const float* shift,
                                     const float* gamma, const float* sum_dy, const float* sum_dy_hhat, float inv_rows,
                                     const float* roww, qagnn_stream_t stream_) {
  hipStream_t stream = (hipStream_t)stream_;
  QAGNN_REQUIRE(dR && Hh && dH && mean && invstd && scale && shift && gamma && sum_dy && sum_dy_hhat, QAGNN_EINVAL,
                "bn_relu_bwd: null pointer");
  QAGNN_REQUIRE(R > 0 && Cc > 0 && Cc % 4 == 0 && ld % 4 == 0, QAGNN_EINVAL, "bn_relu_bwd: bad sizes");
  QAGNN_REQUIRE(ld >= Cc, QAGNN_EINVAL, "bn_relu_bwd: ld=%d below Cc=%d", ld, Cc);
  const int64_t tot = (int64_t)R * (Cc / 4);
  k_bn_relu_bwd<<<cdiv(tot, 256), 256, 0, stream>>>(dR, Hh, dH, ld, R, Cc, mean, invstd, scale, shift, gamma, sum_dy, sum_dy_hhat,
                                                    inv_rows, roww);
  QAGNN_LAUNCH_CHECK("k_bn_relu_bwd");
  return QAGNN_OK;
}

extern "C" int qagnn_bn_finalize_f32(const float* mean, const float* var, const float* gamma, const float* beta, float eps, float* invstd,
                                     float* scale, float* shift, int32_t Cc, float* run_mean, float* run_var, int64_t* num_batches_tracked,
                                     const int64_t* dense_pos, int32_t d, float momentum, float unbias, int32_t ones_col,
                                     qagnn_stream_t stream_) {
  hipStream_t stream = (hipStream_t)stream_;
  QAGNN_REQUIRE(mean && var && gamma && beta && invstd && scale && shift && Cc > 0, QAGNN_EINVAL, "bn_finalize: null pointer");
  QAGNN_REQUIRE(!run_mean || (run_var && dense_pos && d > 0 && d <= Cc), QAGNN_EINVAL, "bn_finalize: running-stat arguments");
  k_bn_finalize<<<cdiv(Cc, 256), 256, 0, stream>>>(mean, var, gamma, beta, eps, invstd, scale, shift, Cc, run_mean, run_var,
                                                   num_batches_tracked, dense_pos, d, momentum, unbias, ones_col);
  QAGNN_LAUNCH_CHECK("k_bn_finalize");
  return QAGNN_OK;
}

namespace qagnn {
int launch_bn_stats_finalize(const float* part, int n_tiles, int R, int Cc, const float* gamma, const float* beta, float eps, float* stats,
                             float* run_mean, float* run_var, int64_t* nbt, int d, float momentum, float unbias, int ones_col, uint32_t* amax_bound,
                             hipStream_t stream) {
  k_bn_stats_finalize<<<cdiv(Cc, BF_COLS), BF_COLS * BF_PARTS, 0, stream>>>(part, n_tiles, R, Cc, gamma, beta, eps, stats, run_mean, run_var, nbt, d,
                                                                            momentum, unbias, ones_col, amax_bound);
  QAGNN_LAUNCH_CHECK("k_bn_stats_finalize");
  return QAGNN_OK;
}
}

extern "C" int qagnn_bn_stats_finalize_f32(const float* part, int32_t n_tiles, int32_t R, int32_t Cc, const float* gamma, const float* beta,
                                           float eps, float* stats, float* run_mean, float* run_var, int64_t* num_batches_tracked,
                                           const int64_t* dense_pos, int32_t d, float momentum, float unbias, int32_t ones_col,
                                           qagnn_stream_t stream_) {
  hipStream_t stream = (hipStream_t)stream_;
  QAGNN_REQUIRE(part && gamma && beta && stats && R > 0 && Cc > 0 && n_tiles == cdiv(R, ST_TILE), QAGNN_EINVAL,
                "bn_stats_finalize: bad arguments (R=%d needs %d tiles of %d rows, got %d)", R, cdiv(R, ST_TILE), ST_TILE, n_tiles);
  QAGNN_REQUIRE(!run_mean || (run_var && d > 0 && d % 4 == 0 && Cc % 4 == 0 && d <= Cc), QAGNN_EINVAL, "bn_stats_finalize: running-stat arguments");
  (void)dense_pos;
  return launch_bn_stats_finalize(part, n_tiles, R, Cc, gamma, beta, eps, stats, run_mean, run_var, num_batches_tracked, d, momentum, unbias, ones_col,
                                  nullptr, stream);
}

__global__ __launch_bounds__(256) void k_gather_multi(qagnn_gather_tabs t, const int* __restrict__ tid, const int* __restrict__ off,
                                                     float* __restrict__ out, int total) {
  __shared__ const float* ps[QAGNN_GATHER_MAX];
  for (int i = threadIdx.x; i < t.n; i += blockDim.x) ps[i] = t.p[i];
  __syncthreads();
  const int i = blockIdx.x * blockDim.x + threadIdx.x;
  if (i >= total) return;
  const int k = tid[i];
  out[i] = k >= 0 ? ps[k][off[i]] : 0.f;
}

__global__ __launch_bounds__(256) void k_gather_multi_sum(qagnn_gather_tabs t, const int* __restrict__ tid, const int* __restrict__ off, int K, int S,
                                                         float* __restrict__ out) {
  __shared__ const float* ps[QAGNN_GATHER_MAX];
  for (int i = threadIdx.x; i < t.n; i += blockDim.x) ps[i] = t.p[i];
  __syncthreads();
  const int s = blockIdx.x * blockDim.x + threadIdx.x;
  if (s >= S) return;
  float acc = 0.f;
  for (int k = 0; k < K; ++k) {
    const int g = tid[(int64_t)k * S + s];
    const float* p = g >= 0 ? ps[g] : nullptr;
    const float v = p != nullptr ? p[off[(int64_t)k * S + s]] : 0.f;
    acc = k == 0 ? v : acc + v;
  }
  out[s] = acc;
// ... 36 lines not shown

extern "C" int qagnn_gelu_dropout_fwd_f32(const float* X, float* Y, int64_t n, float p, uint64_t seed, qagnn_stream_t stream_) {
  hipStream_t stream = (hipStream_t)stream_;
  QAGNN_REQUIRE(X && Y && n > 0 && n % 4 == 0 && aligned16(X) && aligned16(Y), QAGNN_EINVAL, "gelu_dropout_fwd: bad args");
  QAGNN_REQUIRE(p >= 0.f && p < 1.f, QAGNN_EINVAL, "gelu_dropout_fwd: p=%f", p);
  return launch_gelu_dropout(X, nullptr, Y, n, p, seed, nullptr, nullptr, stream);
}

extern "C" int64_t qagnn_gelu_dropout_amax_scratch_elems(int64_t n) { return gelu_amax_scratch_elems(n); }
extern "C" int qagnn_gelu_dropout_fwd_amax_f32(const float* X, float* Y, int64_t n, float p, uint64_t seed, uint32_t* amax, float* scratch,
                                               qagnn_stream_t stream_) {
  QAGNN_REQUIRE(X && Y && amax && scratch && n > 0 && n % 4 == 0 && aligned16(X) && aligned16(Y), QAGNN_EINVAL, "gelu_dropout_fwd_amax: bad args");
  QAGNN_REQUIRE(p >= 0.f && p < 1.f, QAGNN_EINVAL, "gelu_dropout_fwd_amax: p=%f", p);
  return launch_gelu_dropout(X, nullptr, Y, n, p, seed, amax, scratch, (hipStream_t)stream_);
}

extern "C" int qagnn_gelu_dropout_bwd_amax_f32(const float* X, const float* dY, float* dX, int64_t n, float p, uint64_t seed, uint32_t* amax,
                                               float* scratch, qagnn_stream_t stream_) {
  QAGNN_REQUIRE(X && dY && dX && amax && scratch && n > 0 && n % 4 == 0 && aligned16(X) && aligned16(dY) && aligned16(dX), QAGNN_EINVAL,
                "gelu_dropout_bwd_amax: bad args");
  QAGNN_REQUIRE(p >= 0.f && p < 1.f, QAGNN_EINVAL, "gelu_dropout_bwd_amax: p=%f", p);
  return launch_gelu_dropout(X, dY, dX, n, p, seed, amax, scratch, (hipStream_t)stream_);
}

extern "C" int qagnn_gelu_dropout_bwd_f32(const float* X, const float* dY, float* dX, int64_t n, float p, uint64_t seed,
                                          qagnn_stream_t stream_) {
  hipStream_t stream = (hipStream_t)stream_;
  QAGNN_REQUIRE(X && dY && dX && n > 0 && n % 4 == 0 && aligned16(X) && aligned16(dY) && aligned16(dX), QAGNN_EINVAL,
                "gelu_dropout_bwd: bad args");
  QAGNN_REQUIRE(p >= 0.f && p < 1.f, QAGNN_EINVAL, "gelu_dropout_bwd: p=%f", p);
  return launch_gelu_dropout(X, dY, dX, n, p, seed, nullptr, nullptr, stream);
}

extern "C" int qagnn_absmax_f32(const float* x, int64_t n, uint32_t* slot, qagnn_stream_t stream_) {
  QAGNN_REQUIRE(x && slot && n > 0 && n % 4 == 0 && aligned16(x), QAGNN_EINVAL, "absmax: bad arguments");
  const int64_t n4 = n / 4;
  const int grid = (int)(n4 / 256 + 1 < 1024 ? n4 / 256 + 1 : 1024);
  k_absmax<false><<<grid, 256, 0, (hipStream_t)stream_>>>(x, n4, slot);
  QAGNN_LAUNCH_CHECK("k_absmax");
  return QAGNN_OK;
}

int qagnn::launch_amax_reduce(const float* part, int64_t n, uint32_t* slot, hipStream_t stream) {
  const int grid = (int)(n / 1024 + 1 < 64 ? n / 1024 + 1 : 64);
  k_absmax<true><<<grid, 256, 0, stream>>>(part, n, slot);
  QAGNN_LAUNCH_CHECK("k_amax_reduce");
  return QAGNN_OK;
}

extern "C" int qagnn_zero_words(uint32_t* p, int64_t n, qagnn_stream_t stream_) {
  QAGNN_REQUIRE(p && n > 0, QAGNN_EINVAL, "zero_words: bad arguments");
  k_zero_words<<<(int)(n / 256 + 1 < 256 ? n / 256 + 1 : 256), 256, 0, (hipStream_t)stream_>>>(p, n);
  QAGNN_LAUNCH_CHECK("k_zero_words");
  return QAGNN_OK;
}

extern "C" int qagnn_seed_epoch_advance(uint64_t delta, qagnn_stream_t stream_) {
  unsigned long long* w = const_cast<unsigned long long*>(seed_epoch_ptr());
  QAGNN_REQUIRE(w, QAGNN_EHIP, "seed_epoch: cannot resolve the epoch word on this device");
  k_seed_epoch<<<1, 1, 0, (hipStream_t)stream_>>>(w, delta, 1);
  QAGNN_LAUNCH_CHECK("k_seed_epoch");
  return QAGNN_OK;
}

extern "C" int qagnn_seed_epoch_set(uint64_t value, qagnn_stream_t stream_) {
  unsigned long long* w = const_cast<unsigned long long*>(seed_epoch_ptr());
  QAGNN_REQUIRE(w, QAGNN_EHIP, "seed_epoch: cannot resolve the epoch word on this device");
  k_seed_epoch<<<1, 1, 0, (hipStream_t)stream_>>>(w, value, 0);
  QAGNN_LAUNCH_CHECK("k_seed_epoch");
  return QAGNN_OK;
}

extern "C" int qagnn_sin_basis_f32(const float* score, const float* js, float* out, int32_t ldo, int32_t R, int32_t J,
                                   qagnn_stream_t stream_) {
  hipStream_t stream = (hipStream_t)stream_;
  QAGNN_REQUIRE(score && js && out && R > 0 && J > 0 && ldo >= J, QAGNN_EINVAL, "sin_basis: bad args");
  const int64_t tot = (int64_t)R * ldo;
  k_sin_basis<<<cdiv(tot, 256), 256, 0, stream>>>(score, js, out, ldo, R, J);
  QAGNN_LAUNCH_CHECK("k_sin_basis");
  return QAGNN_OK;
}

namespace qagnn {
int launch_bn_relu_bwd_colsum(const float* dR, const float* Hh, float* dH, int ld, int R, int Cc, const float* mean, const float* invstd,
                              const float* scale, const float* shift, const float* gamma, const float* sum_dy, const float* sum_dy_hhat,
                              float inv_rows, const float* roww, float* colsum, float* workspace, uint32_t* amax, hipStream_t stream) {
  dim3 grid(cdiv(Cc, 256), cdiv(R, 4 * cr_wr(R)));
  if (cr_wr(R) == CR_WR_SMALL)
    k_bn_relu_bwd_colsum<CR_WR_SMALL><<<grid, 256, 0, stream>>>(dR, Hh, dH, ld, R, Cc, mean, invstd, scale, shift, gamma, sum_dy, sum_dy_hhat,
                                                                inv_rows, roww, workspace, amax);
  else
    k_bn_relu_bwd_colsum<CR_WR_BIG><<<grid, 256, 0, stream>>>(dR, Hh, dH, ld, R, Cc, mean, invstd, scale, shift, gamma, sum_dy, sum_dy_hhat,
                                                              inv_rows, roww, workspace, amax);
  QAGNN_LAUNCH_CHECK("k_bn_relu_bwd_colsum");
  k_colreduce_final<<<cdiv(Cc, 64), 64 * CF_Q, 0, stream>>>(workspace, colsum, grid.y, Cc, 1.0f);
  QAGNN_LAUNCH_CHECK("k_colreduce_final");
  return QAGNN_OK;
}
}

extern "C" int qagnn_bn_relu_bwd_colsum_f32(const float* dR, const float* Hh, float* dH, int32_t ld, int32_t R, int32_t Cc, const float* mean,
                                            const float* invstd, const float* scale, const float* shift, const float* gamma,
                                            const float* sum_dy, const float* sum_dy_hhat, float inv_rows, const float* roww, float* colsum,
                                            float* workspace, qagnn_stream_t stream_) {
  hipStream_t stream = (hipStream_t)stream_;
  QAGNN_REQUIRE(dR && Hh && dH && mean && invstd && scale && shift && gamma && sum_dy && sum_dy_hhat && colsum && workspace, QAGNN_EINVAL,
                "bn_relu_bwd_colsum: null pointer");
  QAGNN_REQUIRE(R > 0 && Cc > 0 && Cc % 4 == 0 && ld % 4 == 0, QAGNN_EINVAL, "bn_relu_bwd_colsum: bad sizes");
  QAGNN_REQUIRE(ld >= Cc, QAGNN_EINVAL, "bn_relu_bwd_colsum: ld=%d below Cc=%d", ld, Cc);
  return launch_bn_relu_bwd_colsum(dR, Hh, dH, ld, R, Cc, mean, invstd, scale, shift, gamma, sum_dy, sum_dy_hhat, inv_rows, roww, colsum, workspace,
                                   nullptr, stream);
}

namespace qagnn {
__global__ __launch_bounds__(256) void k_node_prep(const float* __restrict__ raw, const int64_t* __restrict__ adj_len,
                                                   const int64_t* __restrict__ node_type, const int64_t* __restrict__ concept_ids, int n,
                                                   float* __restrict__ score, uint8_t* __restrict__ mask, int64_t* __restrict__ ridx,
                                                   int64_t table_rows, int32_t* __restrict__ err) {
  __shared__ double wsum[4];
  __shared__ int wall[4];
  const int g = blockIdx.x, tid = threadIdx.x;
  const int64_t len = adj_len[g];
  const float s0 = -raw[(int64_t)g * n];
  double part = 0.0;
  int unmasked = 0;
  for (int v = tid; v < n; v += 256) {
    const float d = (-raw[(int64_t)g * n + v] - s0) * (v < len ? 1.0f : 0.0f);
    part += (double)fabsf(d);
    unmasked |= !(v >= len || node_type[(int64_t)g * n + v] == 3);
  }
  for (int o = 32; o > 0; o >>= 1) part += __shfl_xor(part, o, 64);
  unmasked = __any(unmasked);
  if ((tid & 63) == 0) { wsum[tid >> 6] = part; wall[tid >> 6] = unmasked; }
  __syncthreads();
  const float total = (float)(wsum[0] + wsum[1] + wsum[2] + wsum[3]);
  const bool all_masked = !(wall[0] | wall[1] | wall[2] | wall[3]);
  const float denom = total / (float)len + 1e-05f;
  for (int v = tid; v < n; v += 256) {
    const int64_t i = (int64_t)g * n + v;
    const float d = (-raw[i] - s0) * (v < len ? 1.0f : 0.0f);
    score[i] = d / denom;
    const bool m = v >= len || node_type[i] == 3;
    mask[i] = (v == 0 && all_masked) ? 0 : (m ? 1 : 0);
    int64_t r = v == 0 ? -1 : concept_ids[i] - 1;
    if (table_rows > 0 && v != 0 && (r < 0 || r >= table_rows)) {
      r = -1;
      if (err) err[0] = 1;
    }
    ridx[i] = r;
  }
}
}

extern "C" int qagnn_node_prep_f32(const float* raw_scores, const int64_t* adj_len, const int64_t* node_type, const int64_t* concept_ids,
                                   int32_t B, int32_t n, float* score, uint8_t* mask, int64_t* ridx, int64_t table_rows, int32_t* err,
                                   qagnn_stream_t stream_) {
  QAGNN_REQUIRE(raw_scores && adj_len && node_type && concept_ids && score && mask && ridx && B > 0 && n > 0, QAGNN_EINVAL, "node_prep: bad arguments");
  qagnn::k_node_prep<<<B, 256, 0, (hipStream_t)stream_>>>(raw_scores, adj_len, node_type, concept_ids, n, score, mask, ridx, table_rows, err);
  QAGNN_LAUNCH_CHECK("k_node_prep");
  return QAGNN_OK;
}
```

qagnn_amd/csrc/graph_prep.hip:

```cpp
#include <stdarg.h>

#include <stdlib.h>

#include "common.h"

namespace qagnn {

static thread_local char g_err[512] = "";
void set_error(const char* fmt, ...) {
  va_list ap;
  va_start(ap, fmt);
  vsnprintf(g_err, sizeof(g_err), fmt, ap);
  va_end(ap);
}

__device__ __forceinline__ int true_edges(const int* __restrict__ E_dev, int E) {
  return E_dev ? min(max(*E_dev, 0), E) : E;
}

__global__ void k_decode_count(const int64_t* __restrict__ edge_index, int64_t ld_edge, const int64_t* __restrict__ edge_type,
                               const int64_t* __restrict__ node_type, int N, int E_cap, const int* __restrict__ E_dev, int R, int T,
                               int* __restrict__ es, int* __restrict__ et, int* __restrict__ ec, int* __restrict__ cnt_s,
                               int* __restrict__ cnt_t, int* __restrict__ err, int block_n) {
  const int e = blockIdx.x * blockDim.x + threadIdx.x;
// ... 370 lines not shown
__global__ __launch_bounds__(1024) void k_chunk_counts(const int* __restrict__ gc_cnt, int* __restrict__ nch, int n) {
  const int i = blockIdx.x * blockDim.x + threadIdx.x;
  if (i < n) nch[i] = (gc_cnt[i] + QAGNN_CLS_CHUNK - 1) / QAGNN_CLS_CHUNK;
}
__global__ __launch_bounds__(1024) void k_scan_pairs(const int* gc_cnt, int* gcptr, const int* nch, int* chunkptr, int n) {
  if (blockIdx.x == 0) block_exclusive_scan(gc_cnt, gcptr, n);
  else block_exclusive_scan(nch, chunkptr, n);
}
__global__ void k_chunk_fill(const int* __restrict__ gcptr, const int* __restrict__ chunkptr, int* __restrict__ chunk_cls,
                             int* __restrict__ chunk_beg, int* __restrict__ chunk_len, int* __restrict__ n_chunks, int C, int n) {
  const int i = blockIdx.x * blockDim.x + threadIdx.x;
  if (i == 0) *n_chunks = chunkptr[n];
  if (i >= n) return;
  const int b = gcptr[i], e = gcptr[i + 1];
  int k = chunkptr[i];
  for (int p = b; p < e; p += QAGNN_CLS_CHUNK, ++k) {
    chunk_cls[k] = i % C;
    chunk_beg[k] = p;
    chunk_len[k] = min(QAGNN_CLS_CHUNK, e - p);
  }
}

static inline void cls_groups(int Ep, int* nblk, int* gb, int* NG) {
  *nblk = cdiv(Ep, CLS_BLK);
  *gb = cdiv(*nblk, QAGNN_CLS_GROUPS) > 1 ? cdiv(*nblk, QAGNN_CLS_GROUPS) : 1;
  *NG = cdiv(*nblk, *gb);
}

static inline int64_t up4(int64_t x) { return (x + 3) & ~(int64_t)3; }

__global__ void k_xcd_partition(const int* __restrict__ rowptr_s, int N, int cap, int balance, int* __restrict__ base) {
  const int nbk = (N + 3) >> 2, lane = threadIdx.x;
  int cand = 0;
  if (lane >= 1 && lane <= 7) {
    if (balance) {
      const long long W = 4ll * rowptr_s[N] - 3ll * N, target = (W * lane + 7) / 8;
      int lo = 0, hi = nbk;
      while (lo < hi) {
        const int mid = (lo + hi) >> 1, nd = min(4 * mid, N);
        if (4ll * rowptr_s[nd] - 3ll * nd >= target) hi = mid; else lo = mid + 1;
      }
      cand = lo;
    } else {
      const int q = nbk >> 3, r = nbk & 7;
      cand = lane < r ? lane * (q + 1) : r * (q + 1) + (lane - r) * q;
    }
  }
  __shared__ int c[8];
  if (lane < 8) c[lane] = cand;
  __syncthreads();
  if (lane == 0) {
    int prev = 0;
    base[0] = 0;
    for (int k = 1; k < 8; ++k) {
      int b = c[k];
      b = min(b, prev + cap);
      b = max(b, nbk - (8 - k) * cap);
      b = max(b, prev);
      base[k] = b;
      prev = b;
    }
    base[8] = nbk;
  }
}

__global__ __launch_bounds__(1024) void k_live_tiles(const int* __restrict__ rowptr_s, const int* __restrict__ rowptr_t, int N, int T,
                                                     int* __restrict__ live, int* __restrict__ rank, int* __restrict__ list,
                                                     int* __restrict__ n_live) {
  for (int t = threadIdx.x; t < T; t += 1024) {
    const int r0 = t * 32, r1 = min(N, r0 + 32);
    live[t] = (rowptr_s[r1] - rowptr_s[r0] != r1 - r0 || rowptr_t[r1] - rowptr_t[r0] != r1 - r0) ? 1 : 0;
  }
  __syncthreads();
  block_exclusive_scan(live, rank, T);
  __syncthreads();
  const int L = rank[T];
  for (int t = threadIdx.x; t < T; t += 1024) {
    const int r = rank[t];
    list[live[t] ? r : L + (t - r)] = t;
  }
  if (threadIdx.x == 0) *n_live = L;
}

__global__ void k_tn_work_table(const int* __restrict__ n_live, int T, int S, int chunk_tiles, int* __restrict__ out) {
  const int u = blockIdx.x * blockDim.x + threadIdx.x;
  const int L = min(max(n_live[0], 0), T);
  const TnWork w = tn_work(S, T, L, chunk_tiles);
  if (u == 0) { out[0] = w.cK; out[1] = w.cM; out[2] = T; out[3] = L; }
  if (u >= S) return;
  const TnSlot s = tn_slot(w, S, T, u);
  int* o = out + 4 + 5 * u;
  o[0] = s.cb; o[1] = s.list; o[2] = s.beg; o[3] = s.cnt; o[4] = s.pslot;
}

__global__ void k_zero16(int4* __restrict__ p, int64_t n16) {
  for (int64_t i = (int64_t)blockIdx.x * blockDim.x + threadIdx.x; i < n16; i += (int64_t)gridDim.x * blockDim.x) p[i] = make_int4(0, 0, 0, 0);
}

}

using namespace qagnn;

static int xcd_partition(qagnn_graph* g, hipStream_t stream) {
  k_xcd_partition<<<1, 64, 0, stream>>>(g->rowptr_s, g->N, edge_xcd_cap(g->N), 1, g->err + 4);
  QAGNN_LAUNCH_CHECK("k_xcd_partition");
  return QAGNN_OK;
}

static int live_tiles(qagnn_graph* g, int32_t* rank, hipStream_t stream) {
  const LiveTiles lt = live_tiles_of(g);
  k_live_tiles<<<1, 1024, 0, stream>>>(g->rowptr_s, g->rowptr_t, g->N, lt.n_tiles, lt.live, rank, lt.list, lt.n_live);
  QAGNN_LAUNCH_CHECK("k_live_tiles");
  return QAGNN_OK;
}

static hipError_t zero_range(void* p, size_t bytes, hipStream_t stream) {
  if (bytes % 16 != 0 || !aligned16(p)) return hipErrorInvalidValue;
  const int64_t n16 = (int64_t)(bytes / 16);
  if (n16 == 0) return hipSuccess;
  int blocks = (int)((n16 + 255) / 256);
  if (blocks > 1024) blocks = 1024;
  k_zero16<<<blocks, 256, 0, stream>>>((int4*)p, n16);
  return hipGetLastError();
}

struct carved {
  int32_t *eid_t, *gc_cnt, *gcptr, *nch, *cnt_s, *cnt_t, *es, *et, *ec, *tmp_s, *tmp_t, *srcpos, *hist, *live_rank;
  int nblk, gb, NG, pairs;
};
static carved carve(qagnn_graph* g, int32_t* storage, int N, int E, int R, int T, int block_n) {
  carved cv;
  const int Ep = E + N, C = R * T * T + T;
  cls_groups(Ep, &cv.nblk, &cv.gb, &cv.NG);
  cv.pairs = cv.NG * C;
  const int maxch = Ep / QAGNN_CLS_CHUNK + cv.pairs + 1;
  int32_t* p = storage;
  auto take = [&](int64_t n) { int32_t* r = p; p += up4(n); return r; };
  g->N = N; g->E = E; g->Ep = Ep; g->R = R; g->T = T; g->C = C; g->max_chunks = maxch; g->block_n = block_n;
  g->n_groups = cv.NG;
  g->rowptr_s = take(N + 1); g->rowptr_t = take(N + 1);
  g->tgt_s = take(Ep); g->src_s = take(Ep); g->cls_s = take(Ep); g->eid_s = take(Ep);
  g->src_t = take(Ep); g->tgt_t = take(Ep); g->cls_t = take(Ep); g->pos_t = take(Ep);
  g->src_c = take(Ep); g->tgt_c = take(Ep); g->pos_c = take(Ep);
  cv.eid_t = take(Ep);
  cv.gc_cnt = take(cv.pairs + 1); cv.gcptr = take(cv.pairs + 1);
  g->chunkptr = take(cv.pairs + 1);
  cv.nch = take(cv.pairs + 1);
  g->cls_count = take(C);
  g->chunk_cls = take(maxch); g->chunk_beg = take(maxch); g->chunk_len = take(maxch);
  g->n_chunks = take(4); g->err = take(16);
  take(4 + 2 * up4(cdiv(N, 32)));
  cv.cnt_s = take(N); cv.cnt_t = take(N);
  cv.es = take(Ep); cv.et = take(Ep); cv.ec = take(Ep);
  cv.tmp_s = take(Ep); cv.tmp_t = take(Ep); cv.srcpos = take(Ep);
  cv.hist = take((int64_t)cv.nblk * C);
  cv.live_rank = take(cdiv(N, 32) + 1);
  return cv;
}

static int class_pass(qagnn_graph* g, int32_t* hist, int32_t* gc_cnt, int32_t* gcptr, int32_t* nch, int nblk, int gb, int NG, int pairs,
                      hipStream_t stream) {
  const int TB = 256, C = g->C;
  const int* Ep = g->rowptr_s + g->N;
  k_cls_hist<<<nblk, 256, C * sizeof(int), stream>>>(g->cls_s, hist, g->cls_count, Ep, C);
  QAGNN_LAUNCH_CHECK("k_cls_hist");
  k_grp_count<<<cdiv(pairs, TB), TB, 0, stream>>>(hist, gc_cnt, nblk, C, gb, NG);
  QAGNN_LAUNCH_CHECK("k_grp_count");
  k_chunk_counts<<<cdiv(pairs, 1024), 1024, 0, stream>>>(gc_cnt, nch, pairs);
  QAGNN_LAUNCH_CHECK("k_chunk_counts");
  k_scan_pairs<<<2, 1024, 0, stream>>>(gc_cnt, gcptr, nch, g->chunkptr, pairs);
  QAGNN_LAUNCH_CHECK("k_scan_pairs");
  k_grp_base<<<cdiv(pairs, TB), TB, 0, stream>>>(hist, gcptr, nblk, C, gb, NG);
  QAGNN_LAUNCH_CHECK("k_grp_base");
  k_cls_scatter<<<nblk, 64, C * sizeof(int), stream>>>(g->cls_s, g->src_s, g->tgt_s, hist, g->src_c, g->tgt_c, g->pos_c, Ep, C);
  QAGNN_LAUNCH_CHECK("k_cls_scatter");
  k_chunk_fill<<<cdiv(pairs, 256), 256, 0, stream>>>(gcptr, g->chunkptr, g->chunk_cls, g->chunk_beg, g->chunk_len, g->n_chunks, C, pairs);
  QAGNN_LAUNCH_CHECK("k_chunk_fill");
  return QAGNN_OK;
}

extern "C" const char* qagnn_last_error(void) { return g_err; }
extern "C" int qagnn_abi_version(void) { return 25; }

extern "C" int64_t qagnn_graph_storage_elems(int32_t N, int32_t E, int32_t R, int32_t T) {
  const int64_t Ep = (int64_t)E + N, C = (int64_t)R * T * T + T;
  int nblk_i, gb, NG;
  cls_groups((int)Ep, &nblk_i, &gb, &NG);
  const int64_t pairs = (int64_t)NG * C;
  const int64_t maxch = Ep / QAGNN_CLS_CHUNK + pairs + 1;
  const int64_t nblk = nblk_i;
  int64_t tot = 0;
  tot += 2 * up4(N + 1);
  tot += 12 * up4(Ep);
  tot += 4 * up4(pairs + 1);
  tot += up4(C);
  tot += 3 * up4(maxch);
  tot += up4(4) + up4(16);
  tot += 2 * up4(N);
  tot += 6 * up4(Ep);
  tot += up4(nblk * C);
  const int64_t tiles = ((int64_t)N + 31) / 32;
  tot += 2 * up4(tiles) + up4(4) + up4(tiles + 1);
  return tot;
}

extern "C" int qagnn_graph_prep(qagnn_graph* g, int32_t* storage, const int64_t* edge_index, const int64_t* edge_type,
                                const int64_t* node_type, int32_t N, int32_t E, int32_t R, int32_t T, qagnn_stream_t stream_) {
  return qagnn_graph_prep_blocked(g, storage, edge_index, edge_type, node_type, N, E, R, T, 0, stream_);
}

static int prep_sorted(const char* who, qagnn_graph* g, int32_t* storage, const int64_t* edge_index, int64_t ld_edge,
                       const int64_t* edge_type, const int64_t* node_type, int32_t N, int32_t E, const int32_t* E_dev, int32_t R,
                       int32_t T, int32_t block_n, hipStream_t stream) {
  QAGNN_REQUIRE(block_n >= 0 && (block_n == 0 || N % block_n == 0), QAGNN_EINVAL, "%s: N=%d is not a multiple of block_n=%d", who, N, block_n);
  QAGNN_REQUIRE(g && storage && node_type, QAGNN_EINVAL, "%s: null pointer", who);
  QAGNN_REQUIRE(N > 0 && E >= 0 && R > 0 && T > 0, QAGNN_EINVAL, "%s: bad sizes N=%d E=%d R=%d T=%d", who, N, E, R, T);
  QAGNN_REQUIRE(E == 0 || (edge_index && edge_type), QAGNN_EINVAL, "%s: null edge arrays with E=%d", who, E);
  QAGNN_REQUIRE(ld_edge >= E, QAGNN_EINVAL, "%s: ld_edge=%lld below the %d edges the arrays are laid out for", who, (long long)ld_edge, E);
  QAGNN_REQUIRE(aligned16(storage), QAGNN_EINVAL, "%s: storage must be 16-byte aligned", who);
  const int64_t Ep64 = (int64_t)E + N, C64 = (int64_t)R * T * T + T;
  QAGNN_REQUIRE(Ep64 < (1ll << 30), QAGNN_EUNSUPPORTED, "%s: E+N=%lld too large", who, (long long)Ep64);
  QAGNN_REQUIRE(C64 <= 8192, QAGNN_EUNSUPPORTED, "%s: %lld edge classes > 8192", who, (long long)C64);
  const int Ep = (int)Ep64;
  carved cv = carve(g, storage, N, E, R, T, block_n);
  int32_t *cnt_s = cv.cnt_s, *cnt_t = cv.cnt_t, *es = cv.es, *et = cv.et, *ec = cv.ec, *tmp_s = cv.tmp_s, *tmp_t = cv.tmp_t;
  int32_t *srcpos = cv.srcpos, *eid_t = cv.eid_t, *hist = cv.hist, *gc_cnt = cv.gc_cnt, *gcptr = cv.gcptr, *nch = cv.nch;
  const int nblk = cv.nblk, gb = cv.gb, NG = cv.NG, pairs = cv.pairs;

  hipError_t he = zero_range(g->cls_count, (size_t)((char*)es - (char*)g->cls_count), stream);
  if (he != hipSuccess) { set_error("%s: k_zero16 failed: %s", who, hipGetErrorString(he)); return QAGNN_EHIP; }
  const int TB = 256;
  k_decode_count<<<cdiv(Ep, TB), TB, 0, stream>>>(edge_index, ld_edge, edge_type, node_type, N, E, E_dev, R, T, es, et, ec, cnt_s, cnt_t,
                                                   g->err, block_n);
  QAGNN_LAUNCH_CHECK("k_decode_count");
  k_scan3<<<2, 1024, 0, stream>>>(cnt_s, g->rowptr_s, N, cnt_t, g->rowptr_t, N, nullptr, nullptr, 0);
  QAGNN_LAUNCH_CHECK("k_scan3");
  k_fill<<<cdiv(Ep, TB), TB, 0, stream>>>(es, et, g->rowptr_s, g->rowptr_t, cnt_s, cnt_t, tmp_s, tmp_t, N, E, E_dev);
  QAGNN_LAUNCH_CHECK("k_fill");
  k_sort_segments<<<cdiv(2 * (int64_t)N, 4), 256, 0, stream>>>(g->rowptr_s, g->rowptr_t, tmp_s, tmp_t, g->eid_s, eid_t, srcpos, N);
  QAGNN_LAUNCH_CHECK("k_sort_segments");
  k_payload<<<cdiv(Ep, TB), TB, 0, stream>>>(es, et, ec, g->eid_s, eid_t, srcpos, g->tgt_s, g->src_s, g->cls_s, g->src_t,
                                              g->tgt_t, g->cls_t, g->pos_t, N, E, E_dev);
  QAGNN_LAUNCH_CHECK("k_payload");
  int rc = xcd_partition(g, stream);
  if (rc != QAGNN_OK) return rc;
  if ((rc = live_tiles(g, cv.live_rank, stream)) != QAGNN_OK) return rc;
  return class_pass(g, hist, gc_cnt, gcptr, nch, nblk, gb, NG, pairs, stream);
}

extern "C" int qagnn_graph_prep_blocked(qagnn_graph* g, int32_t* storage, const int64_t* edge_index, const int64_t* edge_type,
                                        const int64_t* node_type, int32_t N, int32_t E, int32_t R, int32_t T, int32_t block_n,
                                        qagnn_stream_t stream_) {
  return prep_sorted("graph_prep", g, storage, edge_index, E, edge_type, node_type, N, E, nullptr, R, T, block_n, (hipStream_t)stream_);
}

extern "C" int qagnn_graph_prep_cap(qagnn_graph* g, int32_t* storage, const int64_t* edge_index, int64_t ld_edge,
                                    const int64_t* edge_type, const int64_t* node_type, int32_t N, int32_t E_cap, const int32_t* E_dev,
                                    int32_t R, int32_t T, int32_t block_n, qagnn_stream_t stream_) {
  QAGNN_REQUIRE(E_dev, QAGNN_EINVAL, "graph_prep_cap: null edge-count pointer");
  return prep_sorted("graph_prep_cap", g, storage, edge_index, ld_edge, edge_type, node_type, N, E_cap, E_dev, R, T, block_n,
                     (hipStream_t)stream_);
}

template <class Blobs>
static int from_blobs(const char* who, qagnn_graph* g, int32_t* storage, const Blobs src, const int32_t* edge_off, const int64_t* node_type,
                      int32_t B, int32_t n, int32_t E, int32_t R, int32_t T, hipStream_t stream) {
  QAGNN_REQUIRE(B > 0 && n > 0 && E >= 0 && R > 0 && T > 0, QAGNN_EINVAL, "%s: bad sizes B=%d n=%d E=%d R=%d T=%d", who, B, n, E, R, T);
  QAGNN_REQUIRE(n < 65536 && (int64_t)R * T * T < 65536, QAGNN_EUNSUPPORTED, "%s: n=%d or R*T*T=%d does not fit the 16-bit blob fields", who, n, R * T * T);
  QAGNN_REQUIRE((size_t)(2 * (n + 1)) * sizeof(int) <= 64 * 1024, QAGNN_EUNSUPPORTED, "%s: n=%d node slots per sample exceed the LDS scan", who, n);
  QAGNN_REQUIRE(aligned16(storage), QAGNN_EINVAL, "%s: storage must be 16-byte aligned", who);
  const int64_t N64 = (int64_t)B * n, Ep64 = (int64_t)E + N64, C64 = (int64_t)R * T * T + T;
  QAGNN_REQUIRE(Ep64 < (1ll << 30), QAGNN_EUNSUPPORTED, "%s: E+N=%lld too large", who, (long long)Ep64);
  QAGNN_REQUIRE(C64 <= 8192, QAGNN_EUNSUPPORTED, "%s: %lld edge classes > 8192", who, (long long)C64);
  carved cv = carve(g, storage, (int)N64, E, R, T, n);
  hipError_t he = zero_range(g->cls_count, (size_t)((char*)cv.es - (char*)g->cls_count), stream);
  if (he != hipSuccess) { set_error("%s: k_zero16 failed: %s", who, hipGetErrorString(he)); return QAGNN_EHIP; }
  k_blob_assemble<Blobs><<<B, 256, (size_t)(2 * (n + 1)) * sizeof(int), stream>>>(src, edge_off, node_type, n, B, R, T, g->rowptr_s,
                                                                                  g->tgt_s, g->src_s, g->cls_s, g->eid_s, g->rowptr_t, g->src_t,
                                                                                  g->tgt_t, g->cls_t, g->pos_t, g->err);
  QAGNN_LAUNCH_CHECK("k_blob_assemble");
  int rc = xcd_partition(g, stream);
  if (rc != QAGNN_OK) return rc;
  if ((rc = live_tiles(g, cv.live_rank, stream)) != QAGNN_OK) return rc;
  return class_pass(g, cv.hist, cv.gc_cnt, cv.gcptr, cv.nch, cv.nblk, cv.gb, cv.NG, cv.pairs, stream);
}
// ... 48 lines not shown
```

qagnn_amd/csrc/hop.hip:

```cpp
#include "common.h"

#include <mutex>

namespace qagnn {

static inline int64_t up4(int64_t x) { return (x + 3) & ~(int64_t)3; }
static inline int64_t max64(int64_t a, int64_t b) { return a > b ? a : b; }

static inline int hop_stat_tiles(int N) { return cdiv(N, 128); }
static inline bool hop_stat_width(int DP) { return DP > 192 && DP <= 208; }
static int64_t hop_pack_elems(int DP) { return up4((qagnn_gemm_nn_pack_bytes(3 * DP, DP, DP) + 3) / 4); }
static inline int hop_cls_part_rows(const qagnn_graph* g) { return QAGNN_CLS_SLICES * g->C + g->max_chunks; }

struct HopWs {
  float* base;
  int64_t total = 0;
  float* take(int64_t n) { const int64_t o = total; total += up4(n); return base ? base + o : nullptr; }
};
struct HopFwdWs : HopWs {
  const int64_t N, Ep, DP, ampart_elems = max64(N, gelu_amax_scratch_elems(N * DP));
  float* const score = take(Ep * 4);
  float* const crws = take(max64(qagnn_colreduce_workspace_elems(N, DP, 1), hop_stat_tiles(N) * 3 * DP));
  float* const pkws = take(hop_pack_elems(DP));
  float* const ampart = take(ampart_elems);
  static HopFwdWs layout(int N, int Ep, int DP, int , int , float* base) { return {{base}, N, Ep, DP}; }
};
struct HopBwdWs : HopWs {
  const int64_t N, Ep, DP, SP, cls_part_rows;
  struct { float *dout, *dh1, *dkmq; } set[2] = {{take(N * DP), take(N * DP), take(N * 3 * DP)},
                                                 {take(N * DP), take(N * DP), take(N * 3 * DP)}};
  float* const drelu = take(N * DP);
  float* const gab = take(Ep * 4);
  float* const rs = take(N * 4);
  float* const cls_part = take(cls_part_rows * 2 * DP);
  float* const tnws = take(max64(max64(qagnn_gemm_tn_workspace_elems(N, DP, DP), qagnn_gemm_tn_workspace_elems(N, DP, 3 * DP)),
                                 SP > 0 ? qagnn_gemm_tn_workspace_elems(N, DP + SP, 3 * DP) : 0));
  float* const crws = take(qagnn_colreduce_workspace_elems(N, 3 * DP, 4));
  float* const pkws = take(hop_pack_elems(DP));
  float* const ampart = take(max64(3 * N, gelu_amax_scratch_elems(N * DP)));
  static HopBwdWs layout(int N, int Ep, int DP, int SP, int cls_part_rows, float* base) { return {{base}, N, Ep, DP, SP, cls_part_rows}; }
};

static int check_hop(const qagnn_hop_args* h, const char* who, bool bwd = false) {
  QAGNN_REQUIRE(h && h->g, QAGNN_EINVAL, "%s: null argument block / graph", who);
  QAGNN_REQUIRE(h->N == h->g->N && h->N > 0, QAGNN_EINVAL, "%s: N=%d does not match the graph (N=%d)", who, h->N, h->g->N);
  QAGNN_REQUIRE(h->HP > 0 && h->HP % 4 == 0 && h->DP == 4 * h->HP, QAGNN_EINVAL, "%s: DP=%d must be 4*HP (HP=%d)", who, h->DP, h->HP);
  QAGNN_REQUIRE(h->HP <= 64, QAGNN_EUNSUPPORTED, "%s: head pitch HP=%d must be <= 64 (the edge kernels' lane map)", who, h->HP);
  QAGNN_REQUIRE(h->DP % 16 == 0 && h->SP >= 0 && h->SP % 16 == 0, QAGNN_EUNSUPPORTED,
                "%s: DP=%d and SP=%d must be multiples of 16 (GEMM k-tile)", who, h->DP, h->SP);
  QAGNN_REQUIRE(h->T >= 1 && h->T <= 4, QAGNN_EUNSUPPORTED, "%s: %d node types (the type-table gradient handles 1..4)", who, h->T);
  QAGNN_REQUIRE(h->X && h->ntype && h->Wx_t && h->Wx && h->TT && h->EkEm && h->W1t && h->W1 && h->b1 && h->gamma && h->beta &&
                    h->W2t && h->W2 && h->b2,
                QAGNN_EINVAL, "%s: null parameter pointer", who);
  QAGNN_REQUIRE(h->SP == 0 || (h->S && h->Ws_t && h->Ws), QAGNN_EINVAL, "%s: SP=%d but S / Ws_t / Ws missing", who, h->SP);
  QAGNN_REQUIRE(h->KMQ && h->a && h->alpha && h->aggr && h->h1 && h->out && h->stats, QAGNN_EINVAL, "%s: null saved-buffer pointer", who);
  QAGNN_REQUIRE(h->batch_stats || (h->run_mean_p && h->run_var_p), QAGNN_EINVAL, "%s: running statistics missing", who);
  QAGNN_REQUIRE(!h->apply_act || h->y, QAGNN_EINVAL, "%s: apply_act without an output buffer y", who);
  QAGNN_REQUIRE(h->ws, QAGNN_EINVAL, "%s: null workspace", who);
  const int64_t need = bwd ? HopBwdWs::layout(h->N, h->g->Ep, h->DP, h->SP, hop_cls_part_rows(h->g), nullptr).total
                           : HopFwdWs::layout(h->N, h->g->Ep, h->DP, h->SP, 0, nullptr).total;
  QAGNN_REQUIRE(h->ws_elems >= need, QAGNN_EINVAL, "%s: workspace of %lld floats is too small", who, (long long)h->ws_elems);
  return QAGNN_OK;
}

struct HopAmax {
  bool on;
  uint32_t* x;
  uint32_t* s;
  uint32_t* y;
  uint32_t* own;
  bool h1_pass;
};
static bool hop_h2(const qagnn_hop_args* h, bool infer = false) {
  return h->gemm_split >= 2 && h->amax != nullptr && (infer ? !h->batch_stats : h->batch_stats != 0) && nn_rows_packed(h->N);
}
static int hop_pieces(const qagnn_hop_args* h) { return h->gemm_split == 3 ? 1 : 2; }
static void nn_scaled(const qagnn_hop_args* h, qagnn_gemm_nn_args* a, const uint32_t* am1, const uint32_t* am2 = nullptr) {
  a->a_amax1 = am1, a->a_amax2 = am2, a->pieces = hop_pieces(h) == 1 ? 1 : 0;
}
static HopAmax hop_amax_single(const qagnn_hop_args* h, bool infer = false) {
  HopAmax m{hop_h2(h, infer), nullptr, nullptr, nullptr, h->amax, false};
  m.h1_pass = m.on && infer && hop_stat_width(h->DP);
  if (m.on) {
    m.x = h->x_amax ? const_cast<uint32_t*>(h->x_amax) : h->amax + QAGNN_HOP_AM_X;
    m.s = h->s_amax ? const_cast<uint32_t*>(h->s_amax) : h->amax + QAGNN_HOP_AM_S;
    m.y = h->amax + QAGNN_HOP_AM_Y;
  }
  return m;
}
static HopAmax hop_amax_stack(const qagnn_hop_args* hops, int k, int l, bool infer = false) {
  HopAmax m = hop_amax_single(&hops[l], infer);
  if (!m.on) return m;
  if (l > 0 && hop_h2(&hops[l - 1], infer) && hops[l].X == hops[l - 1].y && hops[l - 1].apply_act && !hops[l].x_amax) m.x = hops[l - 1].amax + QAGNN_HOP_AM_Y;
  if (l > 0 && hop_h2(&hops[0], infer) && hops[l].S == hops[0].S && hops[l].SP == hops[0].SP && !hops[l].s_amax)
    m.s = hops[0].s_amax ? const_cast<uint32_t*>(hops[0].s_amax) : hops[0].amax + QAGNN_HOP_AM_S;
  return m;
}

}

using namespace qagnn;

#define HOP_TRY(call)              \
  do {                             \
    int rc__ = (call);             \
    if (rc__ != QAGNN_OK) return rc__; \
  } while (0)

extern "C" int64_t qagnn_hop_fwd_workspace_elems(int32_t N, int32_t Ep, int32_t DP) { return HopFwdWs::layout(N, Ep, DP, 0, 0, nullptr).total; }
extern "C" int64_t qagnn_hop_bwd_workspace_elems(int32_t N, int32_t Ep, int32_t DP, int32_t SP, int32_t cls_part_rows) {
  return HopBwdWs::layout(N, Ep, DP, SP, cls_part_rows, nullptr).total;
}

static int hop_nn(const qagnn_hop_args* h, const qagnn_gemm_nn_args* a, const float* B1n, int ldn1, const float* B2n, int ldn2, float* pkws, qagnn_stream_t stream) {
  return gemm_nn(NnProduct{a, h->gemm_split != 0, B1n, ldn1, B2n, ldn2, pkws, hop_pack_elems(h->DP) * 4}, (hipStream_t)stream);
}
static int hop_tn(const qagnn_hop_args* h, const float* A1, int Ka1, const float* A2, int Ka2, const float* B, int No, float* C, const float* sc,
                  const float* sh, const uint32_t* am_a1, const uint32_t* am_a2, const uint32_t* am_b, float* tnws, qagnn_stream_t stream,
                  const qagnn_graph* g = nullptr) {
  TnProduct p = tn_product(A1, Ka1, Ka1, A2, Ka2, Ka2, B, No, C, No, h->N, No, sc, sh, tnws, am_a1, am_a2, am_b, hop_pieces(h));
  p.g = g;
  return gemm_tn(p, (hipStream_t)stream);
}
// ... 30 lines not shown
    QAGNN_REQUIRE(!h->run_mean || (h->run_var && h->d > 0 && h->d % 4 == 0 && h->d <= DP), QAGNN_EINVAL, "hop_fwd: running-stat arguments");
    HOP_TRY(launch_bn_stats_finalize(w.crws, hop_stat_tiles(N), N, DP, h->gamma, h->beta, h->eps, h->stats, h->run_mean, h->run_var, h->num_batches_tracked,
                                     h->d, h->momentum, unbias, h->ones_col, h1_bound ? am.own + QAGNN_HOP_AM_H1 : nullptr, (hipStream_t)stream));
  } else {
    const float* mean_u = mean;
    const float* var_u = var;
    if (h->batch_stats) {
      const float inv_rows = (float)(1.0 / (double)N);
      HOP_TRY(qagnn_colreduce_f32(0, h->h1, DP, nullptr, DP, N, DP, nullptr, 1, nullptr, nullptr, nullptr, nullptr, nullptr, inv_rows, mean, w.crws,
                                  stream));
      HOP_TRY(qagnn_colreduce_f32(1, h->h1, DP, nullptr, DP, N, DP, nullptr, 1, mean, nullptr, nullptr, nullptr, nullptr, inv_rows, var, w.crws,
                                  stream));
    } else {
      mean_u = h->run_mean_p;
      var_u = h->run_var_p;
    }
    HOP_TRY(qagnn_bn_finalize_f32(mean_u, var_u, h->gamma, h->beta, h->eps, invstd, scale, shift, DP, h->run_mean, h->run_var,
                                  h->num_batches_tracked, h->dense_pos, h->d, h->momentum, unbias, h->ones_col, stream));
  }
  if (am.h1_pass) {
    HOP_TRY(launch_bn_relu_absmax(h->h1, DP, N, DP, scale, shift, am.own + QAGNN_HOP_AM_H1, w.ampart, (hipStream_t)stream));
  }
  qagnn_gemm_nn_args g2 = {};
  g2.A1 = h->h1; g2.lda1 = DP; g2.K1 = DP; g2.B1 = h->W2t; g2.ldb1 = DP; g2.C = h->out; g2.ldc = DP; g2.M = N; g2.No = DP; g2.bias = h->b2;
  g2.a_scale = scale; g2.a_shift = shift;
  if (h1_bound || am.h1_pass) nn_scaled(h, &g2, am.own + QAGNN_HOP_AM_H1);
  HOP_TRY(hop_nn(h, &g2, h->W2, DP, nullptr, 0, w.pkws, stream));
  if (h->apply_act) {
    QAGNN_REQUIRE(h->p_drop >= 0.f && h->p_drop < 1.f, QAGNN_EINVAL, "hop_fwd: p=%f", h->p_drop);
    HOP_TRY(launch_gelu_dropout(h->out, nullptr, h->y, (int64_t)N * DP, h->p_drop, h->seed, am.on ? am.y : nullptr, w.ampart, (hipStream_t)stream));
  }
  return QAGNN_OK;
}

extern "C" int qagnn_hop_fwd_f32(const qagnn_hop_args* h, qagnn_stream_t stream) {
  QAGNN_REQUIRE(h, QAGNN_EINVAL, "hop_fwd: null argument block");
  HOP_TRY(check_hop(h, "hop_fwd"));
  const HopAmax am = hop_amax_single(h);
  if (am.on) HOP_TRY(qagnn_zero_words(h->amax, QAGNN_HOP_AMAX_WORDS, stream));
  return hop_fwd_one(h, am, h->x_amax != nullptr, h->s_amax != nullptr, stream);
}

namespace qagnn {

constexpr int HOP_MAX_DEV = 16, HOP_EV_POOL = 64;
static hipEvent_t g_hop_ev[HOP_MAX_DEV][HOP_EV_POOL];
static bool g_hop_ev_made[HOP_MAX_DEV];
static std::mutex g_hop_ev_mu;

struct SideSync {
  hipStream_t main, side;
  hipEvent_t* ev;
  int next;
  hipEvent_t take() { return ev[next++ % HOP_EV_POOL]; }
};

static int side_sync_init(SideSync* s, hipStream_t main, hipStream_t side) {
  s->main = main;
  s->side = (side && side != main) ? side : nullptr;
  s->ev = nullptr;
  s->next = 0;
  if (!s->side) return QAGNN_OK;
  int dev = 0;
  hipError_t he = hipGetDevice(&dev);
  QAGNN_REQUIRE(he == hipSuccess && dev >= 0 && dev < HOP_MAX_DEV, QAGNN_EHIP, "hop_bwd: device %d outside the event table", dev);
  std::lock_guard<std::mutex> lk(g_hop_ev_mu);
  if (!g_hop_ev_made[dev]) {
    for (int i = 0; i < HOP_EV_POOL; ++i) {
      he = hipEventCreateWithFlags(&g_hop_ev[dev][i], hipEventDisableTiming);
      QAGNN_REQUIRE(he == hipSuccess, QAGNN_EHIP, "hop_bwd: hipEventCreate failed: %s", hipGetErrorString(he));
    }
    g_hop_ev_made[dev] = true;
  }
  s->ev = g_hop_ev[dev];
  return QAGNN_OK;
}
static int stream_after(hipStream_t to, hipStream_t from, hipEvent_t ev) {
  hipError_t he = hipEventRecord(ev, from);
  if (he == hipSuccess) he = hipStreamWaitEvent(to, ev, 0);
  QAGNN_REQUIRE(he == hipSuccess, QAGNN_EHIP, "hop_bwd: stream fork / join failed: %s", hipGetErrorString(he));
  return QAGNN_OK;
}

static int hop_bwd_one(const qagnn_hop_args* h, const HopAmax& am, SideSync* ss, int set, hipEvent_t* done) {
  QAGNN_REQUIRE(h->dy && h->dWx_t && h->dTT && h->dEkEm && h->dW1t && h->db1 && h->dbn && h->dW2t && h->db2, QAGNN_EINVAL,
                "hop_bwd: null gradient pointer");
  QAGNN_REQUIRE(h->SP == 0 || h->dWs_t, QAGNN_EINVAL, "hop_bwd: dWs_t missing");
  const int N = h->N, DP = h->DP, SP = h->SP, Ep = h->g->Ep;
  const HopBwdWs w = HopBwdWs::layout(N, Ep, DP, SP, hop_cls_part_rows(h->g), h->ws);
  float* const bufA = w.set[set].dout, *const bufC = w.set[set].dh1, *const dKMQ = w.set[set].dkmq, *const bufB = w.drelu;
  const float* mean = h->batch_stats ? h->stats : h->run_mean_p;
  const float* invstd = h->stats + 2 * DP, *scale = h->stats + 3 * DP, *shift = h->stats + 4 * DP;
  const qagnn_stream_t stream = (qagnn_stream_t)ss->main;
  const qagnn_stream_t wstream = (qagnn_stream_t)(ss->side ? ss->side : ss->main);

  const float* dout = h->dy;
  const bool h2 = am.on && hop_stat_width(DP);
  uint32_t* const w_dout = h2 ? am.own + QAGNN_HOP_AM_DOUT : nullptr, *const w_dh1 = h2 ? am.own + QAGNN_HOP_AM_DH1 : nullptr, *const w_dkmq = h2 ? am.own + QAGNN_HOP_AM_DKMQ : nullptr;
  const uint32_t* const w_h1 = h2 ? am.own + QAGNN_HOP_AM_H1 : nullptr, *const w_aggr = h2 ? am.own + QAGNN_HOP_AM_AGGR : nullptr;
  if (h->apply_act) {
    HOP_TRY(launch_gelu_dropout(h->out, h->dy, bufA, (int64_t)N * DP, h->p_drop, h->seed, w_dout, w.ampart, (hipStream_t)stream));
    dout = bufA;
  } else if (h2) {
    HOP_TRY(qagnn_absmax_f32(dout, (int64_t)N * DP, w_dout, stream));
  }
  if (h->ones_col < 0)
    HOP_TRY(qagnn_colreduce_f32(0, dout, DP, nullptr, DP, N, DP, nullptr, 1, nullptr, nullptr, nullptr, nullptr, nullptr, 1.0f, h->db2, w.crws, stream));
  if (ss->side) HOP_TRY(stream_after(ss->side, ss->main, ss->take()));
  HOP_TRY(hop_tn(h, h->h1, DP, nullptr, 0, dout, DP, h->dW2t, scale, shift, w_h1, nullptr, w_dout, w.tnws, wstream));
  if (h->ones_col >= 0 && h->db2 != h->dW2t + (int64_t)h->ones_col * DP) {
    hipError_t he = hipMemcpyAsync(h->db2, h->dW2t + (int64_t)h->ones_col * DP, (size_t)DP * sizeof(float), hipMemcpyDeviceToDevice, (hipStream_t)wstream);
    if (he != hipSuccess) { set_error("hop_bwd: db2 copy failed: %s", hipGetErrorString(he)); return QAGNN_EHIP; }
  }
  qagnn_gemm_nn_args gr = {};
  gr.A1 = dout; gr.lda1 = DP; gr.K1 = DP; gr.B1 = h->W2; gr.ldb1 = DP; gr.C = bufB; gr.ldc = DP; gr.M = N; gr.No = DP;
  nn_scaled(h, &gr, w_dout);
  HOP_TRY(hop_nn(h, &gr, h->W2t, DP, nullptr, 0, w.pkws, stream));
  HOP_TRY(qagnn_colreduce_f32(2, bufB, DP, h->h1, DP, N, DP, nullptr, 1, mean, invstd, scale, shift, nullptr, 1.0f, h->dbn, w.crws, stream));
  HOP_TRY(launch_bn_relu_bwd_colsum(bufB, h->h1, bufC, DP, N, DP, mean, invstd, scale, shift, h->gamma, h->dbn, h->dbn + DP,
                                    h->batch_stats ? (float)(1.0 / (double)N) : 0.f, nullptr, h->db1, w.crws, w_dh1, (hipStream_t)stream));
  if (ss->side) HOP_TRY(stream_after(ss->side, ss->main, ss->take()));
  HOP_TRY(hop_tn(h, h->aggr, DP, nullptr, 0, bufC, DP, h->dW1t, nullptr, nullptr, w_aggr, nullptr, w_dh1, w.tnws, wstream));
  qagnn_gemm_nn_args gg = {};
  gg.A1 = bufC; gg.lda1 = DP; gg.K1 = DP; gg.B1 = h->W1; gg.ldb1 = DP; gg.C = bufB; gg.ldc = DP; gg.M = N; gg.No = DP;
  nn_scaled(h, &gg, w_dh1);
  HOP_TRY(hop_nn(h, &gg, h->W1t, DP, nullptr, 0, w.pkws, stream));
  HOP_TRY(launch_edge_attn_bwd(h->g, h->KMQ, 3 * DP, h->EkEm, 2 * DP, h->HP, h->qscale, h->a, h->alpha, bufB, DP, dKMQ, h->dEkEm, w.gab, w.rs, w.cls_part,
                               h2 ? w.ampart : nullptr, w_dkmq, (hipStream_t)stream));
  if (ss->side) HOP_TRY(stream_after(ss->side, ss->main, ss->take()));
  if (SP > 0 && h->dWs_t == h->dWx_t + (int64_t)DP * 3 * DP) {
    HOP_TRY(hop_tn(h, h->X, DP, h->S, SP, dKMQ, 3 * DP, h->dWx_t, nullptr, nullptr, am.x, am.s, w_dkmq, w.tnws, wstream, h->g));
  } else {
    HOP_TRY(hop_tn(h, h->X, DP, nullptr, 0, dKMQ, 3 * DP, h->dWx_t, nullptr, nullptr, am.x, nullptr, w_dkmq, w.tnws, wstream));
    if (SP > 0) HOP_TRY(hop_tn(h, h->S, SP, nullptr, 0, dKMQ, 3 * DP, h->dWs_t, nullptr, nullptr, am.s, nullptr, w_dkmq, w.tnws, wstream));
  }
  if (SP > 0 && h->tab_col >= 0) {
    QAGNN_REQUIRE(h->tab_col + h->T <= SP, QAGNN_EINVAL, "hop_bwd: tab_col=%d + T=%d exceeds SP=%d", h->tab_col, h->T, SP);
    if (h->dTT != h->dWs_t + (int64_t)h->tab_col * 3 * DP) {
      hipError_t he = hipMemcpyAsync(h->dTT, h->dWs_t + (int64_t)h->tab_col * 3 * DP, (size_t)h->T * 3 * DP * sizeof(float), hipMemcpyDeviceToDevice,
                                     (hipStream_t)wstream);
      if (he != hipSuccess) { set_error("hop_bwd: dTT copy failed: %s", hipGetErrorString(he)); return QAGNN_EHIP; }
    }
  } else {
    HOP_TRY(qagnn_colreduce_f32(0, dKMQ, 3 * DP, nullptr, 3 * DP, N, 3 * DP, h->ntype, h->T, nullptr, nullptr, nullptr, nullptr, nullptr, 1.0f, h->dTT,
                                w.crws, stream));
  }
  if (ss->side) {
    *done = ss->take();
    hipError_t he = hipEventRecord(*done, ss->side);
    QAGNN_REQUIRE(he == hipSuccess, QAGNN_EHIP, "hop_bwd: hipEventRecord failed: %s", hipGetErrorString(he));
  }
  if (h->dX) {
    qagnn_gemm_nn_args gx = {};
    gx.A1 = dKMQ; gx.lda1 = 3 * DP; gx.K1 = 3 * DP; gx.B1 = h->Wx; gx.ldb1 = DP; gx.C = h->dX; gx.ldc = DP; gx.M = N; gx.No = DP;
    gx.accumulate = h->accumulate_dX;
    nn_scaled(h, &gx, w_dkmq);
    HOP_TRY(hop_nn(h, &gx, h->Wx_t, 3 * DP, nullptr, 0, w.pkws, stream));
  }
  if (SP > 0 && h->dS) {
    qagnn_gemm_nn_args gs = {};
    gs.A1 = dKMQ; gs.lda1 = 3 * DP; gs.K1 = 3 * DP; gs.B1 = h->Ws; gs.ldb1 = SP; gs.C = h->dS; gs.ldc = SP; gs.M = N; gs.No = SP;
    gs.accumulate = h->accumulate_dS;
    nn_scaled(h, &gs, w_dkmq);
    HOP_TRY(hop_nn(h, &gs, h->Ws_t, 3 * DP, nullptr, 0, w.pkws, stream));
  }
  return QAGNN_OK;
}

static_assert(QAGNN_HOP_AM_DH1 == QAGNN_HOP_AM_DOUT + 1 && QAGNN_HOP_AM_DKMQ == QAGNN_HOP_AM_DOUT + 2, "the backward's words are three in a row");
__global__ void k_zero_bwd_words(uint32_t* __restrict__ amax, int k) {
  for (int i = threadIdx.x; i < 3 * k; i += blockDim.x) amax[(i / 3) * QAGNN_HOP_AMAX_WORDS + QAGNN_HOP_AM_DOUT + i % 3] = 0u;
}
static int zero_bwd_words(const qagnn_hop_args* hops, int k, hipStream_t main) {
  bool all = true, any = false, one_array = true;
  for (int l = 0; l < k; ++l) {
    const bool h2 = hop_amax_stack(hops, k, l).on && hop_stat_width(hops[l].DP);
    all = all && h2;
    any = any || h2;
    one_array = one_array && hops[l].amax != nullptr && hops[l].amax == hops[0].amax + (int64_t)l * QAGNN_HOP_AMAX_WORDS;
  }
  if (!any) return QAGNN_OK;
  if (all && one_array) {
    k_zero_bwd_words<<<1, 64, 0, main>>>(hops[0].amax, k);
    QAGNN_LAUNCH_CHECK("k_zero_bwd_words");
    return QAGNN_OK;
  }
  for (int l = 0; l < k; ++l)
    if (hop_amax_stack(hops, k, l).on && hop_stat_width(hops[l].DP))
      HOP_TRY(qagnn_zero_words(hops[l].amax + QAGNN_HOP_AM_DOUT, 3, (qagnn_stream_t)main));
  return QAGNN_OK;
}

static int stack_bwd_impl(const qagnn_hop_args* hops, int k, hipStream_t main) {
  for (int l = 0; l < k; ++l) HOP_TRY(check_hop(&hops[l], k > 1 ? "stack_bwd" : "hop_bwd", true));
  HOP_TRY(zero_bwd_words(hops, k, main));
  SideSync ss;
  HOP_TRY(side_sync_init(&ss, main, (hipStream_t)hops[k - 1].side_stream));
  hipEvent_t done[2] = {nullptr, nullptr};
  int rc = QAGNN_OK;
  for (int it = 0, l = k - 1; l >= 0 && rc == QAGNN_OK; --l, ++it) {
    const int set = it & 1;
    if (ss.side && done[set]) {
      hipError_t he = hipStreamWaitEvent(ss.main, done[set], 0);
      if (he != hipSuccess) { set_error("stack_bwd: hipStreamWaitEvent failed: %s", hipGetErrorString(he)); rc = QAGNN_EHIP; break; }
    }
    rc = hop_bwd_one(&hops[l], hop_amax_stack(hops, k, l), &ss, set, &done[set]);
  }
  if (ss.side) {
    hipEvent_t ev = ss.take();
    hipError_t he = hipEventRecord(ev, ss.side);
    if (he == hipSuccess) he = hipStreamWaitEvent(ss.main, ev, 0);
    if (he != hipSuccess && rc == QAGNN_OK) { set_error("stack_bwd: joining the weight-gradient stream failed: %s", hipGetErrorString(he)); rc = QAGNN_EHIP; }
  }
  return rc;
}

}

extern "C" int qagnn_hop_bwd_f32(const qagnn_hop_args* h, qagnn_stream_t stream) {
  QAGNN_REQUIRE(h, QAGNN_EINVAL, "hop_bwd: null argument block");
  return stack_bwd_impl(h, 1, (hipStream_t)stream);
}

static int stack_fwd_impl(const qagnn_hop_args* hops, int32_t k, bool infer, qagnn_stream_t stream) {
  bool any = false, one_array = true;
  for (int l = 0; l < k; ++l) {
    any = any || hop_h2(&hops[l], infer);
    one_array = one_array && hops[l].amax != nullptr && hops[l].amax == hops[0].amax + (int64_t)l * QAGNN_HOP_AMAX_WORDS;
  }
  if (any && one_array) HOP_TRY(qagnn_zero_words(hops[0].amax, (int64_t)k * QAGNN_HOP_AMAX_WORDS, stream));
  for (int l = 0; l < k; ++l) {
    const HopAmax am = hop_amax_stack(hops, k, l, infer);
    if (am.on && !one_array) HOP_TRY(qagnn_zero_words(hops[l].amax, QAGNN_HOP_AMAX_WORDS, stream));
    HOP_TRY(hop_fwd_one(&hops[l], am, am.on && am.x != hops[l].amax + QAGNN_HOP_AM_X, am.on && am.s != hops[l].amax + QAGNN_HOP_AM_S, stream));
  }
  return QAGNN_OK;
}

extern "C" int qagnn_stack_fwd_f32(const qagnn_hop_args* hops, int32_t k, qagnn_stream_t stream) {
  QAGNN_REQUIRE(hops && k > 0, QAGNN_EINVAL, "stack_fwd: no hops");
  for (int l = 0; l < k; ++l) HOP_TRY(check_hop(&hops[l], "stack_fwd"));
  return stack_fwd_impl(hops, k, false, stream);
}

extern "C" int qagnn_stack_infer_f32(const qagnn_hop_args* hops, int32_t k, qagnn_stream_t stream) {
  QAGNN_REQUIRE(hops && k > 0, QAGNN_EINVAL, "stack_infer: no hops");
  for (int l = 0; l < k; ++l) {
    const qagnn_hop_args* h = &hops[l];
    HOP_TRY(check_hop(h, "stack_infer"));
    QAGNN_REQUIRE(!h->batch_stats && h->run_mean_p && h->run_var_p, QAGNN_EINVAL, "stack_infer: hop %d asks for batch statistics", l);
    QAGNN_REQUIRE(!h->run_mean && !h->run_var && !h->num_batches_tracked, QAGNN_EINVAL, "stack_infer: hop %d would update running statistics", l);
    QAGNN_REQUIRE(h->p_drop == 0.f, QAGNN_EINVAL, "stack_infer: hop %d has dropout p=%f", l, h->p_drop);
    const int64_t row = (int64_t)h->N * h->DP * 4, edges = (int64_t)h->g->Ep * 16;
    const struct { const void* p; int64_t bytes; } wr[] = {{h->KMQ, 3 * row}, {h->a, edges}, {h->alpha, edges}, {h->aggr, row}, {h->h1, row},
                                                           {h->out, row}, {h->stats, (int64_t)5 * h->DP * 4}, {h->apply_act ? h->y : nullptr, row}};
    const struct { const void* p; int64_t bytes; } rd[] = {{h->X, row}, {h->SP > 0 ? h->S : nullptr, (int64_t)h->N * h->SP * 4}};
    for (const auto& w : wr)
      for (const auto& r : rd) {
        const char* const wp = (const char*)w.p, *const rp = (const char*)r.p;
        QAGNN_REQUIRE(!wp || !rp || wp + w.bytes <= rp || rp + r.bytes <= wp, QAGNN_EINVAL,
                      "stack_infer: hop %d writes into one of its own inputs (y over X, or X / S inside its result buffers)", l);
      }
    QAGNN_REQUIRE(qagnn_bn_relu_absmax_scratch_elems(h->N, h->DP) <= HopFwdWs::layout(h->N, h->g->Ep, h->DP, h->SP, 0, nullptr).ampart_elems, QAGNN_EINVAL,
                  "stack_infer: the partial maxima of bn_relu_absmax do not fit the hop workspace");
  }
  return stack_fwd_impl(hops, k, true, stream);
}

extern "C" int qagnn_stack_bwd_f32(const qagnn_hop_args* hops, int32_t k, qagnn_stream_t stream) {
  QAGNN_REQUIRE(hops && k > 0, QAGNN_EINVAL, "stack_bwd: no hops");
  return stack_bwd_impl(hops, k, (hipStream_t)stream);
}
```

Before: 45060 QA-subgraphs/s.

## Defer per-layer class and db1 column reductions to one batched launch after stack backward

The per-relation-class reduction of dEkEm and the final db1 column reduction for each GAT layer are no longer launched inside each hop's backward. Partials for every layer now go into a stacked deferral workspace and are reduced once, after all hops finish, by layer-batched kernels. The class reduce also gains a live-class list built at graph prep, so empty classes are skipped, and the amax fold moves into k_edge_bwd_cls. The aim is fewer small serial launches on the critical backward path, at the cost of extra workspace per layer and more ABI surface.

New measurement: 45950 QA-subgraphs/s (median of 6 runs). 1.02x the previous value.

```diff
diff --git a/__graft_entry__.py b/__graft_entry__.py
--- a/__graft_entry__.py
+++ b/__graft_entry__.py
@@ -12,7 +12,7 @@
     from qagnn_amd import _lib
     lib = _lib.load_library(path)
     assert lib.qagnn_abi_version() == _lib.ABI_VERSION
-    for name in _lib.EXPORTS + _lib.EXPORTS_TN + _lib.EXPORTS_INFER + _lib.EXPORTS_LOSS + _lib.EXPORTS_EXPLAIN:
+    for name in _lib.EXPORTS + _lib.EXPORTS_TN + _lib.EXPORTS_INFER + _lib.EXPORTS_LOSS + _lib.EXPORTS_EXPLAIN + _lib.EXPORTS_DEFER:
         assert hasattr(lib, name), name
     import qagnn_amd.modeling_qagnn
     import oracle.qagnn_oracle
diff --git a/include/qagnn_hip_defer.h b/include/qagnn_hip_defer.h
--- /dev/null
+++ b/include/qagnn_hip_defer.h
@@ -0,0 +1,22 @@
+#ifndef QAGNN_HIP_DEFER_H
+#define QAGNN_HIP_DEFER_H
+
+#include "qagnn_hip.h"
+
+#ifdef __cplusplus
+extern "C" {
+#endif
+
+int qagnn_defer_version(void);
+
+int64_t qagnn_stack_bwd_defer_elems(int32_t N, int32_t DP, int32_t cls_part_rows, int32_t k);
+
+#define QAGNN_DEFER_MAX_HOPS 16
+
+int qagnn_stack_bwd_deferred_f32(const qagnn_hop_args* hops, int32_t k, float* defer_ws, int64_t defer_elems, qagnn_stream_t stream);
+
+#ifdef __cplusplus
+}
+#endif
+
+#endif
diff --git a/qagnn_amd/_lib.py b/qagnn_amd/_lib.py
--- a/qagnn_amd/_lib.py
+++ b/qagnn_amd/_lib.py
@@ -26,6 +26,8 @@
                  'qagnn_choice_eval_f32']
 EXPORTS_LOSS = ['qagnn_loss_version', 'qagnn_choice_loss_f32', 'qagnn_choice_loss_bwd_f32']
 EXPORTS_EXPLAIN = ['qagnn_explain_version', 'qagnn_attn_export_f32', 'qagnn_attn_trace_f32']
+EXPORTS_DEFER = ['qagnn_defer_version', 'qagnn_stack_bwd_defer_elems', 'qagnn_stack_bwd_deferred_f32']
+DEFER_MAX_HOPS = 16
 TRACE_MAX_N = 1024
 LOSS_KINDS = {'cross_entropy': 0, 'margin_rank': 1}
 LOSS_THREADS = 256
@@ -185,7 +187,11 @@
     lib.qagnn_explain_version.argtypes = []
     lib.qagnn_attn_export_f32.argtypes = [C.POINTER(qagnn_graph), _vp, _i64, _i32, _vp, _i64, _vp]
     lib.qagnn_attn_trace_f32.argtypes = [C.POINTER(qagnn_graph), _vp, _i64, _i32, _i32, _i32, _i32, _i32, _vp, _vp, _vp, _vp]
-    for name in EXPORTS + EXPORTS_TN + EXPORTS_INFER + EXPORTS_LOSS + EXPORTS_EXPLAIN:
+    lib.qagnn_defer_version.argtypes = []
+    lib.qagnn_stack_bwd_defer_elems.restype = _i64
+    lib.qagnn_stack_bwd_defer_elems.argtypes = [_i32, _i32, _i32, _i32]
+    lib.qagnn_stack_bwd_deferred_f32.argtypes = [C.POINTER(qagnn_hop_args), _i32, _vp, _i64, _vp]
+    for name in EXPORTS + EXPORTS_TN + EXPORTS_INFER + EXPORTS_LOSS + EXPORTS_EXPLAIN + EXPORTS_DEFER:
         fn = getattr(lib, name)
         if fn.restype is C.c_int and name not in ('qagnn_abi_version',):
             fn.restype = _i32
@@ -313,6 +319,11 @@
         T4 = (T + 3) // 4 * 4
         w = self.array('err', 16 + 4 + 2 * T4)[16:]
         return w[4:4 + T], w[4 + T4:4 + T4 + T], w[:1]
+
+    def live_classes(self):
+        T4 = ((self.N + 31) // 32 + 3) // 4 * 4
+        w = self.array('err', 16 + 4 + 2 * T4 + 4 + self.C)[16 + 4 + 2 * T4:]
+        return w[4:4 + self.C], w[:1]
 
     @property
     def cls_part_rows(self):
@@ -1283,7 +1294,7 @@
         return ys[k - 1], (KMQ, aa, rows, stats, amax, x_amax if x_amax is not None else ext, s_amax if s_amax is not None else ext)
 
     def stack_bwd(self, graph, HP, qscale, X, S, ntype, prms, batch_stats, eps, p, seeds, saved, dy, need_dX, need_dS, dX_acc=None, tab_col=-1,
-                  overlap=True):
+                  overlap=True, defer=True):
         k = len(prms)
         KMQ, aa, rows, stats = saved[:4]
         p_amax = saved[4].data_ptr() if len(saved) > 4 else None
@@ -1313,5 +1324,9 @@
                 h.dX, h.accumulate_dX = dX.data_ptr(), (1 if dX_acc is not None else 0)
             if dS is not None:
                 h.dS, h.accumulate_dS = dS.data_ptr(), (0 if l == k - 1 else 1)
-        self._check(self.lib.qagnn_stack_bwd_f32(hops, k, self._stream()), 'qagnn_stack_bwd_f32')
+        if defer and k <= DEFER_MAX_HOPS:
+            dws = torch.empty(self.lib.qagnn_stack_bwd_defer_elems(N, DP, graph.cls_part_rows, k), dtype=torch.float32, device=dev)
+            self._check(self.lib.qagnn_stack_bwd_deferred_f32(hops, k, dws.data_ptr(), dws.numel(), self._stream()), 'qagnn_stack_bwd_deferred_f32')
+        else:
+            self._check(self.lib.qagnn_stack_bwd_f32(hops, k, self._stream()), 'qagnn_stack_bwd_f32')
         return dX, dS, grads
diff --git a/qagnn_amd/build.py b/qagnn_amd/build.py
--- a/qagnn_amd/build.py
+++ b/qagnn_amd/build.py
@@ -17,7 +17,8 @@
                                                                  os.path.join(HERE, '..', 'include', 'qagnn_hip_tn.h'),
                                                                  os.path.join(HERE, '..', 'include', 'qagnn_hip_infer.h'),
                                                                  os.path.join(HERE, '..', 'include', 'qagnn_hip_loss.h'),
-                                                                 os.path.join(HERE, '..', 'include', 'qagnn_hip_explain.h')]
+                                                                 os.path.join(HERE, '..', 'include', 'qagnn_hip_explain.h'),
+                                                                 os.path.join(HERE, '..', 'include', 'qagnn_hip_defer.h')]
 
 
 def source_hash():
diff --git a/qagnn_amd/csrc/common.h b/qagnn_amd/csrc/common.h
--- a/qagnn_amd/csrc/common.h
+++ b/qagnn_amd/csrc/common.h
@@ -142,13 +142,23 @@
   int32_t* const p = g->err + 16;
   return LiveTiles{T, p, p + 4, p + 4 + T4};
 }
+struct LiveClasses { int32_t *n_live, *list; };
+inline LiveClasses live_classes_of(const qagnn_graph* g) {
+  const LiveTiles lt = live_tiles_of(g);
+  int32_t* const p = lt.list + ((lt.n_tiles + 3) & ~3);
+  return LiveClasses{p, p + 4};
+}
 
 int launch_gelu_dropout(const float* X, const float* dY, float* out, int64_t n, float p, uint64_t seed, uint32_t* amax, float* amax_part,
                         hipStream_t stream);
 int64_t gelu_amax_scratch_elems(int64_t n);
 int launch_bn_relu_bwd_colsum(const float* dR, const float* Hh, float* dH, int ld, int R, int Cc, const float* mean, const float* invstd,
                               const float* scale, const float* shift, const float* gamma, const float* sum_dy, const float* sum_dy_hhat,
-                              float inv_rows, const float* roww, float* colsum, float* workspace, uint32_t* amax, hipStream_t stream);
+                              float inv_rows, const float* roww, float* colsum, float* workspace, uint32_t* amax, bool finalize, hipStream_t stream);
+constexpr int DEFER_LAYERS_MAX = 16;
+struct LayerOut { float* p[DEFER_LAYERS_MAX]; };
+int64_t bn_colsum_part_elems(int R, int Cc);
+int launch_colreduce_final_layers(const float* part, int64_t layer_stride, int layers, const LayerOut& outs, int R, int Cc, hipStream_t stream);
 int launch_bn_stats_finalize(const float* part, int n_tiles, int R, int Cc, const float* gamma, const float* beta, float eps, float* stats,
                              float* run_mean, float* run_var, int64_t* nbt, int d, float momentum, float unbias, int ones_col, uint32_t* amax_bound,
                              hipStream_t stream);
@@ -157,7 +167,9 @@
                          float* score, float* a, float* alpha, float* aggr, int32_t lda, float* amax_part , hipStream_t stream);
 int launch_edge_attn_bwd(const qagnn_graph* g, const float* KMQ, int32_t ldk, const float* EkEm, int32_t lde, int32_t HP, float qscale,
                          const float* a, const float* alpha, const float* G, int32_t ldg, float* dKMQ, float* dEkEm, float* ga, float* rs,
-                         float* cls_part, float* amax_part , uint32_t* amax_slot, hipStream_t stream);
+                         float* cls_part, float* amax_part , uint32_t* amax_slot, bool reduce_now, hipStream_t stream);
+int launch_cls_reduce(const qagnn_graph* g, int32_t HP, float* cls_part, int64_t layer_stride, int layers, const LayerOut& out, int32_t lde,
+                      hipStream_t stream);
 int launch_amax_reduce(const float* part, int64_t n, uint32_t* slot, hipStream_t stream);
 int launch_bn_relu_absmax(const float* H, int ldh, int R, int Cc, const float* scale, const float* shift, uint32_t* slot, float* part, hipStream_t stream);
 
diff --git a/qagnn_amd/csrc/edge_attn.hip b/qagnn_amd/csrc/edge_attn.hip
--- a/qagnn_amd/csrc/edge_attn.hip
+++ b/qagnn_amd/csrc/edge_attn.hip
@@ -376,13 +376,24 @@
   if (amax_part) node_amax(L.act ? absmax4(dK) : 0.f, amax_part, t);
 }
 
+constexpr int CLS_AMAX_BLOCKS = 64;
 __global__ __launch_bounds__(256) void k_edge_bwd_cls(const int* __restrict__ n_chunks, const int* __restrict__ chunk_beg,
                                                       const int* __restrict__ chunk_len, const int* __restrict__ src_c,
                                                       const int* __restrict__ tgt_c, const int* __restrict__ pos_c,
                                                       const float* __restrict__ KMQ, int ldk, int HP,
                                                       const float* __restrict__ alpha, const float* __restrict__ gsb,
-                                                      const float* __restrict__ G, int ldg, float* __restrict__ cls_part, int N) {
+                                                      const float* __restrict__ G, int ldg, float* __restrict__ cls_part, int N,
+                                                      const float* __restrict__ amax_part, int npart, uint32_t* __restrict__ amax_slot) {
   __shared__ float4 slab[2][4][SLAB_ROWS];
+  if (amax_part) {
+    const int nfold = min((int)gridDim.x, CLS_AMAX_BLOCKS);
+    if ((int)blockIdx.x < nfold) {
+      __shared__ float red[16];
+      float m = 0.f;
+      for (int i = blockIdx.x * 256 + threadIdx.x; i < npart; i += nfold * 256) m = fmaxf(m, amax_part[i]);
+      block_amax_merge(m, amax_slot, red);
+    }
+  }
   const int nch = *n_chunks, nb_real = (nch + 3) >> 2;
   if ((int)blockIdx.x >= nb_real) return;
   const int k = __builtin_amdgcn_readfirstlane(xcd_remap(blockIdx.x, nb_real) * 4 + (threadIdx.x >> 6));
@@ -424,11 +435,15 @@
   }
 }
 
-__global__ __launch_bounds__(1024) void k_cls_reduce(const int* __restrict__ chunkptr, const float* __restrict__ cls_part,
-                                                     float* __restrict__ slices, int DP2, int C, int NG) {
+__global__ __launch_bounds__(1024) void k_cls_reduce(const int* __restrict__ n_live, const int* __restrict__ live_cls,
+                                                     const int* __restrict__ chunkptr, const float* __restrict__ cls_part,
+                                                     float* __restrict__ slices, int64_t layer_stride, int DP2, int C, int NG) {
   extern __shared__ float4 sm4[];
   __shared__ int cp_lo[QAGNN_CLS_GROUPS], cp_hi[QAGNN_CLS_GROUPS];
-  const int c = blockIdx.x, sl = blockIdx.y;
+  if ((int)blockIdx.x >= min(*n_live, C)) return;
+  const int c = __builtin_amdgcn_readfirstlane(live_cls[blockIdx.x]), sl = blockIdx.y;
+  cls_part += (int64_t)blockIdx.z * layer_stride;
+  slices += (int64_t)blockIdx.z * layer_stride;
   if (threadIdx.x < NG) {
     cp_lo[threadIdx.x] = chunkptr[threadIdx.x * C + c];
     cp_hi[threadIdx.x] = chunkptr[threadIdx.x * C + c + 1];
@@ -455,24 +470,20 @@
     st4(slices + ((int64_t)c * QAGNN_CLS_SLICES + sl) * DP2 + threadIdx.x * 4, s);
   }
 }
-__global__ __launch_bounds__(256) void k_cls_reduce2(const float* __restrict__ slices, float* __restrict__ dEkEm, int lde, int DP2, int C,
-                                                     const float* __restrict__ amax_part, int npart, uint32_t* __restrict__ amax_slot) {
+__global__ __launch_bounds__(256) void k_cls_reduce2(const float* __restrict__ slices, int64_t layer_stride, const int* __restrict__ cls_count,
+                                                     const LayerOut out, int lde, int DP2, int C) {
   const int ncol4 = DP2 >> 2;
   const int i = blockIdx.x * blockDim.x + threadIdx.x;
-  if (i < C * ncol4) {
-    const int c = i / ncol4, col4 = i - c * ncol4;
-    const float* p = slices + (int64_t)c * QAGNN_CLS_SLICES * DP2 + col4 * 4;
-    float4 s = ld4(p);
+  if (i >= C * ncol4) return;
+  const int c = i / ncol4, col4 = i - c * ncol4;
+  float4 s = zero4();
+  if (cls_count[c] > 0) {
+    const float* p = slices + (int64_t)blockIdx.y * layer_stride + (int64_t)c * QAGNN_CLS_SLICES * DP2 + col4 * 4;
+    s = ld4(p);
 #pragma unroll
     for (int q = 1; q < QAGNN_CLS_SLICES; ++q) s = add4(s, ld4(p + (int64_t)q * DP2));
-    st4(dEkEm + (int64_t)c * lde + col4 * 4, s);
-  }
-  if (amax_part) {
-    __shared__ float red[16];
-    float m = 0.f;
-    for (int k = i; k < npart; k += (int)(gridDim.x * blockDim.x)) m = fmaxf(m, amax_part[k]);
-    block_amax_merge(m, amax_slot, red);
-  }
+  }
+  st4(out.p[blockIdx.y] + (int64_t)c * lde + col4 * 4, s);
 }
 
 static int check_common(const qagnn_graph* g, const float* KMQ, int ldk, const float* EkEm, int lde, int HP, const char* who) {
@@ -516,12 +527,12 @@
 extern "C" int qagnn_edge_attn_bwd_f32(const qagnn_graph* g, const float* KMQ, int32_t ldk, const float* EkEm, int32_t lde,
                                        int32_t HP, float qscale, const float* a, const float* alpha, const float* G, int32_t ldg,
                                        float* dKMQ, float* dEkEm, float* ga, float* rs, float* cls_part, qagnn_stream_t stream_) {
-  return launch_edge_attn_bwd(g, KMQ, ldk, EkEm, lde, HP, qscale, a, alpha, G, ldg, dKMQ, dEkEm, ga, rs, cls_part, nullptr, nullptr, (hipStream_t)stream_);
+  return launch_edge_attn_bwd(g, KMQ, ldk, EkEm, lde, HP, qscale, a, alpha, G, ldg, dKMQ, dEkEm, ga, rs, cls_part, nullptr, nullptr, true, (hipStream_t)stream_);
 }
 
 int qagnn::launch_edge_attn_bwd(const qagnn_graph* g, const float* KMQ, int32_t ldk, const float* EkEm, int32_t lde, int32_t HP, float qscale,
                                 const float* a, const float* alpha, const float* G, int32_t ldg, float* dKMQ, float* dEkEm, float* ga, float* rs,
-                                float* cls_part, float* amax_part, uint32_t* amax_slot, hipStream_t stream) {
+                                float* cls_part, float* amax_part, uint32_t* amax_slot, bool reduce_now, hipStream_t stream) {
   TimedScope timed(3, stream);
   int rc = check_common(g, KMQ, ldk, EkEm, lde, HP, "edge_attn_bwd");
   if (rc != QAGNN_OK) return rc;
@@ -539,15 +550,30 @@
   k_edge_bwd_tgt<<<nb, 256, 0, stream>>>(g->rowptr_t, g->src_t, g->pos_t, KMQ, ldk, HP, ga, dKMQ, g->N, g->err + 4, amax_part ? amax_part + 2 * (int64_t)g->N : nullptr);
   QAGNN_LAUNCH_CHECK("k_edge_bwd_tgt");
   k_edge_bwd_cls<<<cdiv(g->max_chunks, 4), 256, 0, stream>>>(g->n_chunks, g->chunk_beg, g->chunk_len, g->src_c, g->tgt_c, g->pos_c,
-                                                             KMQ, ldk, HP, alpha, ga, G, ldg, cls_part, g->N);
+                                                             KMQ, ldk, HP, alpha, ga, G, ldg, cls_part, g->N, amax_slot ? amax_part : nullptr,
+                                                             3 * g->N, amax_slot);
   QAGNN_LAUNCH_CHECK("k_edge_bwd_cls");
+  if (!reduce_now) return QAGNN_OK;
+  LayerOut out = {};
+  out.p[0] = dEkEm;
+  return launch_cls_reduce(g, HP, cls_part, 0, 1, out, lde, stream);
+}
+
+int qagnn::launch_cls_reduce(const qagnn_graph* g, int32_t HP, float* cls_part, int64_t layer_stride, int layers, const LayerOut& out, int32_t lde,
+                             hipStream_t stream) {
+  TimedScope timed(3, stream);
+  QAGNN_REQUIRE(g && cls_part && layers >= 1 && layers <= DEFER_LAYERS_MAX, QAGNN_EINVAL, "cls_reduce: %d layers (1..%d)", layers, DEFER_LAYERS_MAX);
+  QAGNN_REQUIRE(HP > 0 && HP % 4 == 0 && HP <= 64 && lde >= 8 * HP && lde % 4 == 0 && layer_stride % 4 == 0, QAGNN_EINVAL, "cls_reduce: bad pitch");
+  for (int l = 0; l < layers; ++l) QAGNN_REQUIRE(out.p[l] && aligned16(out.p[l]), QAGNN_EINVAL, "cls_reduce: bad output pointer of layer %d", l);
+  const int DP2 = 8 * HP;
   const int cr_threads = g->Ep < 65536 && DP2 / 4 <= 128 ? 256 : 1024;
   const int P = cr_threads / (DP2 / 4);
+  const LiveClasses lc = live_classes_of(g);
   float* slices = cls_part + (int64_t)g->max_chunks * DP2;
-  k_cls_reduce<<<dim3(g->C, QAGNN_CLS_SLICES), cr_threads, (size_t)P * (DP2 / 4) * sizeof(float4), stream>>>(g->chunkptr, cls_part, slices, DP2,
-                                                                                                          g->C, g->n_groups);
+  k_cls_reduce<<<dim3(g->C, QAGNN_CLS_SLICES, layers), cr_threads, (size_t)P * (DP2 / 4) * sizeof(float4), stream>>>(
+      lc.n_live, lc.list, g->chunkptr, cls_part, slices, layer_stride, DP2, g->C, g->n_groups);
   QAGNN_LAUNCH_CHECK("k_cls_reduce");
-  k_cls_reduce2<<<cdiv((int64_t)g->C * (DP2 / 4), 256), 256, 0, stream>>>(slices, dEkEm, lde, DP2, g->C, amax_slot ? amax_part : nullptr, 3 * g->N, amax_slot);
+  k_cls_reduce2<<<dim3(cdiv((int64_t)g->C * (DP2 / 4), 256), layers), 256, 0, stream>>>(slices, layer_stride, g->cls_count, out, lde, DP2, g->C);
   QAGNN_LAUNCH_CHECK("k_cls_reduce2");
   return QAGNN_OK;
 }
diff --git a/qagnn_amd/csrc/elementwise.hip b/qagnn_amd/csrc/elementwise.hip
--- a/qagnn_amd/csrc/elementwise.hip
+++ b/qagnn_amd/csrc/elementwise.hip
@@ -81,11 +81,13 @@
 }
 
 constexpr int CF_Q = 16;
-__global__ __launch_bounds__(64 * CF_Q) void k_colreduce_final(const float* __restrict__ part, float* __restrict__ out, int nchunks,
+__global__ __launch_bounds__(64 * CF_Q) void k_colreduce_final(const float* __restrict__ part, int64_t layer_stride, const LayerOut outs, int nchunks,
                                                                int tot, float out_scale) {
   __shared__ float red[CF_Q][64];
   const int lane = threadIdx.x & 63, q = threadIdx.x >> 6;
   const int o = blockIdx.x * 64 + lane;
+  part += (int64_t)blockIdx.y * layer_stride;
+  float* const __restrict__ out = outs.p[blockIdx.y];
   float s0 = 0.f, s1 = 0.f;
   if (o < tot) {
     int c = q;
@@ -409,7 +411,7 @@
   }
   QAGNN_LAUNCH_CHECK("k_colreduce");
   const int tot = nout * Cc;
-  k_colreduce_final<<<cdiv(tot, 64), 64 * CF_Q, 0, stream>>>(workspace, out, grid.y, tot, out_scale);
+  k_colreduce_final<<<cdiv(tot, 64), 64 * CF_Q, 0, stream>>>(workspace, 0, LayerOut{{out}}, grid.y, tot, out_scale);
   QAGNN_LAUNCH_CHECK("k_colreduce_final");
   return QAGNN_OK;
 }
@@ -612,9 +614,17 @@
 }
 
 namespace qagnn {
+int64_t bn_colsum_part_elems(int R, int Cc) { return (int64_t)cdiv(R, 4 * cr_wr(R)) * Cc; }
+int launch_colreduce_final_layers(const float* part, int64_t layer_stride, int layers, const LayerOut& outs, int R, int Cc, hipStream_t stream) {
+  QAGNN_REQUIRE(part && layers >= 1 && layers <= DEFER_LAYERS_MAX && layer_stride >= 0, QAGNN_EINVAL, "colreduce_final: %d layers", layers);
+  for (int l = 0; l < layers; ++l) QAGNN_REQUIRE(outs.p[l], QAGNN_EINVAL, "colreduce_final: null output of layer %d", l);
+  k_colreduce_final<<<dim3(cdiv(Cc, 64), layers), 64 * CF_Q, 0, stream>>>(part, layer_stride, outs, cdiv(R, 4 * cr_wr(R)), Cc, 1.0f);
+  QAGNN_LAUNCH_CHECK("k_colreduce_final");
+  return QAGNN_OK;
+}
 int launch_bn_relu_bwd_colsum(const float* dR, const float* Hh, float* dH, int ld, int R, int Cc, const float* mean, const float* invstd,
                               const float* scale, const float* shift, const float* gamma, const float* sum_dy, const float* sum_dy_hhat,
-                              float inv_rows, const float* roww, float* colsum, float* workspace, uint32_t* amax, hipStream_t stream) {
+                              float inv_rows, const float* roww, float* colsum, float* workspace, uint32_t* amax, bool finalize, hipStream_t stream) {
   dim3 grid(cdiv(Cc, 256), cdiv(R, 4 * cr_wr(R)));
   if (cr_wr(R) == CR_WR_SMALL)
     k_bn_relu_bwd_colsum<CR_WR_SMALL><<<grid, 256, 0, stream>>>(dR, Hh, dH, ld, R, Cc, mean, invstd, scale, shift, gamma, sum_dy, sum_dy_hhat,
@@ -623,9 +633,8 @@
     k_bn_relu_bwd_colsum<CR_WR_BIG><<<grid, 256, 0, stream>>>(dR, Hh, dH, ld, R, Cc, mean, invstd, scale, shift, gamma, sum_dy, sum_dy_hhat,
                                                               inv_rows, roww, workspace, amax);
   QAGNN_LAUNCH_CHECK("k_bn_relu_bwd_colsum");
-  k_colreduce_final<<<cdiv(Cc, 64), 64 * CF_Q, 0, stream>>>(workspace, colsum, grid.y, Cc, 1.0f);
-  QAGNN_LAUNCH_CHECK("k_colreduce_final");
-  return QAGNN_OK;
+  if (!finalize) return QAGNN_OK;
+  return launch_colreduce_final_layers(workspace, 0, 1, LayerOut{{colsum}}, R, Cc, stream);
 }
 }
 
@@ -639,7 +648,7 @@
   QAGNN_REQUIRE(R > 0 && Cc > 0 && Cc % 4 == 0 && ld % 4 == 0, QAGNN_EINVAL, "bn_relu_bwd_colsum: bad sizes");
   QAGNN_REQUIRE(ld >= Cc, QAGNN_EINVAL, "bn_relu_bwd_colsum: ld=%d below Cc=%d", ld, Cc);
   return launch_bn_relu_bwd_colsum(dR, Hh, dH, ld, R, Cc, mean, invstd, scale, shift, gamma, sum_dy, sum_dy_hhat, inv_rows, roww, colsum, workspace,
-                                   nullptr, stream);
+                                   nullptr, true, stream);
 }
 
 namespace qagnn {
diff --git a/qagnn_amd/csrc/graph_prep.hip b/qagnn_amd/csrc/graph_prep.hip
--- a/qagnn_amd/csrc/graph_prep.hip
+++ b/qagnn_amd/csrc/graph_prep.hip
@@ -476,6 +476,29 @@
   if (threadIdx.x == 0) *n_live = L;
 }
 
+__global__ __launch_bounds__(1024) void k_live_classes(const int* __restrict__ cls_count, int C, int* __restrict__ list, int* __restrict__ n_live) {
+  __shared__ int wc[16];
+  const int lane = threadIdx.x & 63, w = threadIdx.x >> 6;
+  const unsigned long long lt = lane == 0 ? 0ull : (~0ull >> (64 - lane));
+  int base = 0;
+  for (int c0 = 0; c0 < C; c0 += 1024) {
+    const int c = c0 + (int)threadIdx.x;
+    const bool live = c < C && cls_count[c] > 0;
+    const unsigned long long m = __ballot(live);
+    if (lane == 0) wc[w] = __builtin_popcountll(m);
+    __syncthreads();
+    int off = base, tot = 0;
+    for (int i = 0; i < 16; ++i) {
+      if (i < w) off += wc[i];
+      tot += wc[i];
+    }
+    if (live) list[off + __builtin_popcountll(m & lt)] = c;
+    base += tot;
+    __syncthreads();
+  }
+  if (threadIdx.x == 0) *n_live = base;
+}
+
 __global__ void k_tn_work_table(const int* __restrict__ n_live, int T, int S, int chunk_tiles, int* __restrict__ out) {
   const int u = blockIdx.x * blockDim.x + threadIdx.x;
   const int L = min(max(n_live[0], 0), T);
@@ -544,6 +567,7 @@
   g->chunk_cls = take(maxch); g->chunk_beg = take(maxch); g->chunk_len = take(maxch);
   g->n_chunks = take(4); g->err = take(16);
   take(4 + 2 * up4(cdiv(N, 32)));
+  take(4 + up4(C));
   cv.cnt_s = take(N); cv.cnt_t = take(N);
   cv.es = take(Ep); cv.et = take(Ep); cv.ec = take(Ep);
   cv.tmp_s = take(Ep); cv.tmp_t = take(Ep); cv.srcpos = take(Ep);
@@ -558,6 +582,9 @@
   const int* Ep = g->rowptr_s + g->N;
   k_cls_hist<<<nblk, 256, C * sizeof(int), stream>>>(g->cls_s, hist, g->cls_count, Ep, C);
   QAGNN_LAUNCH_CHECK("k_cls_hist");
+  const LiveClasses lc = live_classes_of(g);
+  k_live_classes<<<1, 1024, 0, stream>>>(g->cls_count, C, lc.list, lc.n_live);
+  QAGNN_LAUNCH_CHECK("k_live_classes");
   k_grp_count<<<cdiv(pairs, TB), TB, 0, stream>>>(hist, gc_cnt, nblk, C, gb, NG);
   QAGNN_LAUNCH_CHECK("k_grp_count");
   k_chunk_counts<<<cdiv(pairs, 1024), 1024, 0, stream>>>(gc_cnt, nch, pairs);
@@ -595,6 +622,7 @@
   tot += up4(nblk * C);
   const int64_t tiles = ((int64_t)N + 31) / 32;
   tot += 2 * up4(tiles) + up4(4) + up4(tiles + 1);
+  tot += up4(4) + up4(C);
   return tot;
 }
 
diff --git a/qagnn_amd/csrc/hop.hip b/qagnn_amd/csrc/hop.hip
--- a/qagnn_amd/csrc/hop.hip
+++ b/qagnn_amd/csrc/hop.hip
@@ -1,4 +1,5 @@
 #include "common.h"
+#include "../../include/qagnn_hip_defer.h"
 
 #include <mutex>
 
@@ -39,6 +40,14 @@
   float* const pkws = take(hop_pack_elems(DP));
   float* const ampart = take(max64(3 * N, gelu_amax_scratch_elems(N * DP)));
   static HopBwdWs layout(int N, int Ep, int DP, int SP, int cls_part_rows, float* base) { return {{base}, N, Ep, DP, SP, cls_part_rows}; }
+};
+
+struct StackDeferWs : HopWs {
+  const int64_t N, DP, cls_part_rows, k;
+  const int64_t cls_stride = up4(cls_part_rows * 2 * DP), db1_stride = up4(bn_colsum_part_elems((int)N, (int)DP));
+  float* const cls_part = take(k * cls_stride);
+  float* const db1_part = take(k * db1_stride);
+  static StackDeferWs layout(int N, int DP, int cls_part_rows, int k, float* base) { return {{base}, N, DP, cls_part_rows, k}; }
 };
 
 static int check_hop(const qagnn_hop_args* h, const char* who, bool bwd = false) {
@@ -235,7 +244,7 @@
   return QAGNN_OK;
 }
 
-static int hop_bwd_one(const qagnn_hop_args* h, const HopAmax& am, SideSync* ss, int set, hipEvent_t* done) {
+static int hop_bwd_one(const qagnn_hop_args* h, const HopAmax& am, SideSync* ss, int set, hipEvent_t* done, const StackDeferWs* d = nullptr, int l = 0) {
   QAGNN_REQUIRE(h->dy && h->dWx_t && h->dTT && h->dEkEm && h->dW1t && h->db1 && h->dbn && h->dW2t && h->db2, QAGNN_EINVAL,
                 "hop_bwd: null gradient pointer");
   QAGNN_REQUIRE(h->SP == 0 || h->dWs_t, QAGNN_EINVAL, "hop_bwd: dWs_t missing");
@@ -271,15 +280,16 @@
   HOP_TRY(hop_nn(h, &gr, h->W2t, DP, nullptr, 0, w.pkws, stream));
   HOP_TRY(qagnn_colreduce_f32(2, bufB, DP, h->h1, DP, N, DP, nullptr, 1, mean, invstd, scale, shift, nullptr, 1.0f, h->dbn, w.crws, stream));
   HOP_TRY(launch_bn_relu_bwd_colsum(bufB, h->h1, bufC, DP, N, DP, mean, invstd, scale, shift, h->gamma, h->dbn, h->dbn + DP,
-                                    h->batch_stats ? (float)(1.0 / (double)N) : 0.f, nullptr, h->db1, w.crws, w_dh1, (hipStream_t)stream));
+                                    h->batch_stats ? (float)(1.0 / (double)N) : 0.f, nullptr, h->db1, d ? d->db1_part + l * d->db1_stride : w.crws, w_dh1,
+                                    d == nullptr, (hipStream_t)stream));
   if (ss->side) HOP_TRY(stream_after(ss->side, ss->main, ss->take()));
   HOP_TRY(hop_tn(h, h->aggr, DP, nullptr, 0, bufC, DP, h->dW1t, nullptr, nullptr, w_aggr, nullptr, w_dh1, w.tnws, wstream));
   qagnn_gemm_nn_args gg = {};
   gg.A1 = bufC; gg.lda1 = DP; gg.K1 = DP; gg.B1 = h->W1; gg.ldb1 = DP; gg.C = bufB; gg.ldc = DP; gg.M = N; gg.No = DP;
   nn_scaled(h, &gg, w_dh1);
   HOP_TRY(hop_nn(h, &gg, h->W1t, DP, nullptr, 0, w.pkws, stream));
-  HOP_TRY(launch_edge_attn_bwd(h->g, h->KMQ, 3 * DP, h->EkEm, 2 * DP, h->HP, h->qscale, h->a, h->alpha, bufB, DP, dKMQ, h->dEkEm, w.gab, w.rs, w.cls_part,
-                               h2 ? w.ampart : nullptr, w_dkmq, (hipStream_t)stream));
+  HOP_TRY(launch_edge_attn_bwd(h->g, h->KMQ, 3 * DP, h->EkEm, 2 * DP, h->HP, h->qscale, h->a, h->alpha, bufB, DP, dKMQ, h->dEkEm, w.gab, w.rs,
+                               d ? d->cls_part + l * d->cls_stride : w.cls_part, h2 ? w.ampart : nullptr, w_dkmq, d == nullptr, (hipStream_t)stream));
   if (ss->side) HOP_TRY(stream_after(ss->side, ss->main, ss->take()));
   if (SP > 0 && h->dWs_t == h->dWx_t + (int64_t)DP * 3 * DP) {
     HOP_TRY(hop_tn(h, h->X, DP, h->S, SP, dKMQ, 3 * DP, h->dWx_t, nullptr, nullptr, am.x, am.s, w_dkmq, w.tnws, wstream, h->g));
@@ -344,8 +354,25 @@
   return QAGNN_OK;
 }
 
-static int stack_bwd_impl(const qagnn_hop_args* hops, int k, hipStream_t main) {
+static_assert(DEFER_LAYERS_MAX == QAGNN_DEFER_MAX_HOPS, "the header states the pointer table's length");
+static bool stack_defers(const qagnn_hop_args* hops, int k) {
+  if (k > DEFER_LAYERS_MAX) return false;
+  for (int l = 1; l < k; ++l)
+    if (hops[l].g != hops[0].g || hops[l].N != hops[0].N || hops[l].DP != hops[0].DP || hops[l].HP != hops[0].HP) return false;
+  return true;
+}
+
+static int stack_bwd_impl(const qagnn_hop_args* hops, int k, hipStream_t main, float* defer_ws = nullptr, int64_t defer_elems = 0) {
   for (int l = 0; l < k; ++l) HOP_TRY(check_hop(&hops[l], k > 1 ? "stack_bwd" : "hop_bwd", true));
+  const bool defer = defer_ws != nullptr;
+  QAGNN_REQUIRE(!defer || stack_defers(hops, k), QAGNN_EUNSUPPORTED,
+                "stack_bwd: a deferral workspace with %d hops that do not share one graph, N, DP and HP, or with more than %d hops", k, DEFER_LAYERS_MAX);
+  const StackDeferWs dws = defer ? StackDeferWs::layout(hops[0].N, hops[0].DP, hop_cls_part_rows(hops[0].g), k, defer_ws) : StackDeferWs::layout(0, 0, 0, 0, nullptr);
+  if (defer) {
+    QAGNN_REQUIRE(aligned16(defer_ws) && defer_elems >= dws.total, QAGNN_EINVAL, "stack_bwd: deferral workspace of %lld floats is too small (%lld) or unaligned",
+                  (long long)defer_elems, (long long)dws.total);
+    for (int l = 0; l < k; ++l) QAGNN_REQUIRE(hops[l].dEkEm && hops[l].db1, QAGNN_EINVAL, "stack_bwd: null gradient pointer");
+  }
   HOP_TRY(zero_bwd_words(hops, k, main));
   SideSync ss;
   HOP_TRY(side_sync_init(&ss, main, (hipStream_t)hops[k - 1].side_stream));
@@ -357,7 +384,13 @@
       hipError_t he = hipStreamWaitEvent(ss.main, done[set], 0);
       if (he != hipSuccess) { set_error("stack_bwd: hipStreamWaitEvent failed: %s", hipGetErrorString(he)); rc = QAGNN_EHIP; break; }
     }
-    rc = hop_bwd_one(&hops[l], hop_amax_stack(hops, k, l), &ss, set, &done[set]);
+    rc = hop_bwd_one(&hops[l], hop_amax_stack(hops, k, l), &ss, set, &done[set], defer ? &dws : nullptr, l);
+  }
+  if (defer && rc == QAGNN_OK) {
+    LayerOut cls = {}, db1 = {};
+    for (int l = 0; l < k; ++l) cls.p[l] = hops[l].dEkEm, db1.p[l] = hops[l].db1;
+    rc = launch_cls_reduce(hops[0].g, hops[0].HP, dws.cls_part, dws.cls_stride, k, cls, 2 * hops[0].DP, main);
+    if (rc == QAGNN_OK) rc = launch_colreduce_final_layers(dws.db1_part, dws.db1_stride, k, db1, hops[0].N, hops[0].DP, main);
   }
   if (ss.side) {
     hipEvent_t ev = ss.take();
@@ -424,3 +457,12 @@
   QAGNN_REQUIRE(hops && k > 0, QAGNN_EINVAL, "stack_bwd: no hops");
   return stack_bwd_impl(hops, k, (hipStream_t)stream);
 }
+
+extern "C" int qagnn_defer_version(void) { return 1; }
+extern "C" int64_t qagnn_stack_bwd_defer_elems(int32_t N, int32_t DP, int32_t cls_part_rows, int32_t k) {
+  return N > 0 && DP > 0 && cls_part_rows >= 0 && k > 0 ? StackDeferWs::layout(N, DP, cls_part_rows, k, nullptr).total : 0;
+}
+extern "C" int qagnn_stack_bwd_deferred_f32(const qagnn_hop_args* hops, int32_t k, float* defer_ws, int64_t defer_elems, qagnn_stream_t stream) {
+  QAGNN_REQUIRE(hops && k > 0, QAGNN_EINVAL, "stack_bwd: no hops");
+  return stack_bwd_impl(hops, k, (hipStream_t)stream, defer_ws, defer_elems);
+}
```
